# cosdata/cosdata

Measured on AMD Instinct MI355X. Metric: QPS at recall@10≥0.95, 1024-dim dense cosine, 1/2/4/8 MI355X, higher is better.
Workload: dtype u8

## Files before the change

cosdata_amd/_lib.py:

```python
from __future__ import annotations

import ctypes as C
import os
import subprocess

_PKG = os.path.dirname(os.path.abspath(__file__))
SO_PATH = os.path.join(_PKG, "libcosdata_hip.so")
CSRC = os.path.join(_PKG, "csrc")

OK, ERR_STORAGE_MISMATCH, ERR_CALCULATION, ERR_INVALID, ERR_UNIMPLEMENTED, ERR_HIP, ERR_NOT_READY, ERR_NO_DEVICE = range(8)
STATUS_NAMES = {
    0: "OK", 1: "StorageMismatch", 2: "CalculationError", 3: "Invalid", 4: "Unimplemented", 5: "HipError",
    6: "NotReady", 7: "NoDevice",
}
ABI_VERSION = 1


class CosdataError(RuntimeError):

    def __init__(self, status: int, message: str):
        super().__init__(f"[{STATUS_NAMES.get(status, status)}] {message}")
        self.status = status


class CosParams(C.Structure):
    _fields_ = [
        ("struct_size", C.c_uint32), ("abi_version", C.c_uint32), ("dim", C.c_uint32), ("metric", C.c_uint32),
        ("storage", C.c_uint32), ("resolution", C.c_uint32), ("range_lo", C.c_float), ("range_hi", C.c_float),
        ("num_layers", C.c_uint32), ("neighbors_count", C.c_uint32), ("level0_neighbors_count", C.c_uint32),
        ("ef_construction", C.c_uint32), ("ef_search", C.c_uint32), ("shortlist_size", C.c_uint32),
        ("visited_mode", C.c_uint32), ("device", C.c_int32), ("id_base", C.c_uint32), ("reserved", C.c_uint32),
        ("seed", C.c_uint64),
    ]


class CosSearchStats(C.Structure):
    _fields_ = [
        ("evals", C.c_uint64), ("expansions", C.c_uint64), ("adj_bytes", C.c_uint64), ("rerank_rows", C.c_uint64),
        ("walk_ms", C.c_float), ("finalize_ms", C.c_float), ("prep_ms", C.c_float), ("reserved", C.c_uint32),
    ]


class CosWalkSplit(C.Structure):
    _fields_ = [
        ("struct_size", C.c_uint32), ("queries", C.c_uint32), ("table_level_min", C.c_uint32), ("table_cols", C.c_uint32),
        ("cut_after_level", C.c_uint32), ("reserved", C.c_uint32),
        ("table_ms", C.c_float), ("upper_ms", C.c_float), ("sort_ms", C.c_float), ("lower_ms", C.c_float),
        ("table_int8_ops", C.c_double), ("table_evals", C.c_uint64),
        ("upper_evals", C.c_uint64), ("upper_expansions", C.c_uint64), ("upper_adj_bytes", C.c_uint64),
        ("lower_evals", C.c_uint64), ("lower_expansions", C.c_uint64), ("lower_adj_bytes", C.c_uint64),
    ]


class CosTimingSummary(C.Structure):
    _fields_ = [("launches", C.c_uint32), ("prep_ms_sum", C.c_float), ("walk_ms_sum", C.c_float), ("finalize_ms_sum", C.c_float),
                ("walk_ms_min", C.c_float), ("walk_ms_max", C.c_float)]


class CosCoalescingStats(C.Structure):
    _fields_ = [("launches", C.c_uint64), ("queries", C.c_uint64), ("requests", C.c_uint64), ("closed_full", C.c_uint64),
                ("closed_quiet", C.c_uint64), ("closed_deadline", C.c_uint64), ("solo_calls", C.c_uint64)]


class CosSparseStats(C.Structure):
    _fields_ = [("kernel_ms", C.c_float), ("blocks", C.c_uint32), ("postings_visited", C.c_uint64), ("posting_bytes", C.c_uint64)]


class CosFlatStats(C.Structure):
    _fields_ = [("gemm_ms", C.c_float), ("gemm_launches", C.c_uint32), ("int8_ops", C.c_double), ("code_bytes", C.c_double)]


class CosBM25Stats(C.Structure):
    _fields_ = [("struct_size", C.c_uint32), ("documents_count", C.c_uint32), ("n_terms", C.c_uint32), ("largest_doc_id", C.c_uint32),
                ("dir_rows", C.c_uint32), ("dir_tiles", C.c_uint32), ("reserved", C.c_uint32),
                ("postings", C.c_uint64), ("tombstones", C.c_uint64), ("device_bytes", C.c_uint64)]


class CosSparseIndexStats(C.Structure):
    _fields_ = [("struct_size", C.c_uint32), ("n_vectors", C.c_uint32), ("n_dims", C.c_uint32), ("dir_rows", C.c_uint32),
                ("dir_tiles", C.c_uint32), ("packed", C.c_uint32), ("have_raw", C.c_uint32), ("reserved", C.c_uint32),
                ("postings", C.c_uint64), ("removed", C.c_uint64), ("raw_pairs", C.c_uint64), ("device_bytes", C.c_uint64)]


def build(force: bool = False, verbose: bool = False) -> str:
    srcs = [os.path.join(CSRC, f) for f in os.listdir(CSRC) if f.endswith((".hip", ".h"))]
    srcs.append(os.path.join(_PKG, "..", "include", "cosdata_hip.h"))
    stale = force or not os.path.exists(SO_PATH) or any(os.path.getmtime(s) > os.path.getmtime(SO_PATH) for s in srcs)
    if force:
        subprocess.check_call(["make", "-C", CSRC, "-s", "clean"])
    if stale:
        cmd = ["make", "-C", CSRC, "-j", str(max(2, min(16, 2 * (os.cpu_count() or 1))))]
        if not verbose:
            cmd.append("-s")
        subprocess.check_call(cmd)
    return SO_PATH


_lib = None

ABI_SYMBOLS = [
    "cos_index_create", "cos_index_destroy", "cos_last_error_string", "cos_device_count",
    "cos_index_upload_vectors", "cos_index_set_root", "cos_index_upload_graph_level", "cos_index_level_count",
    "cos_index_download_graph_level", "cos_index_download_codes", "cos_index_download_root", "cos_index_build", "cos_index_append", "cos_index_delete", "cos_index_restore_link_state", "cos_index_release_link_state", "cos_index_enable_metadata", "cos_index_upload_meta_nodes", "cos_index_upload_meta_graph_level", "cos_index_build_meta", "cos_index_meta_level_count", "cos_index_download_meta_graph_level", "cos_search_filtered_batch",
    "cos_ann_search_filtered_batch", "cos_index_load_reference_dir", "cos_reference_dir_level_counts", "cos_reference_dir_read_level",
    "cos_search_batch", "cos_search_batch_device", "cos_ann_search_batch", "cos_index_set_coalescing", "cos_index_coalescing_stats", "cos_index_set_ef_search",
    "cos_index_set_visited_mode", "cos_index_set_latency_mode", "cos_index_set_latency_waves", "cos_index_set_walk_order", "cos_index_walk_order_cuts", "cos_index_set_walk_table", "cos_index_walk_table_info", "cos_index_last_walk_split", "cos_index_enable_timing", "cos_index_last_stats", "cos_index_timing_summary", "cos_quantize_batch",
    "cos_code_bytes", "cos_sample_values_range", "cos_distance_batch", "cos_bruteforce_topk", "cos_flat_search_batch", "cos_bm25_create", "cos_bm25_destroy",
    "cos_bm25_insert", "cos_bm25_delete", "cos_bm25_stats", "cos_bm25_download",
    "cos_bm25_search_batch", "cos_bm25_search_batch_device", "cos_rrf_fuse_batch", "cos_hybrid_search_batch", "cos_text_process", "cos_text_count_tokens", "cos_bm25_term_frequency", "cos_xxhash32", "cos_stem_english", "cos_sparse_create", "cos_sparse_build_csr", "cos_sparse_create_from_vectors", "cos_sparse_destroy", "cos_sparse_search_batch", "cos_sparse_last_stats", "cos_sparse_layout",
    "cos_sparse_set_max_candidates", "cos_sparse_max_candidates",
    "cos_sparse_insert", "cos_sparse_delete", "cos_sparse_stats", "cos_sparse_download", "cos_merge_topk_device", "cos_merge_topk_packed_device", "cos_hbm_probe",
    "cos_shardset_unique_id", "cos_shardset_create", "cos_shardset_destroy", "cos_shardset_search_batch", "cos_shardset_exchange_device",
    "cos_tuning_set", "cos_tuning_clear", "cos_tuning_get",
]


def lib():
    global _lib
    if _lib is not None:
        return _lib
    if not os.path.exists(SO_PATH):
        raise CosdataError(ERR_NO_DEVICE, f"{SO_PATH} is missing: build it with `python -c 'import __graft_entry__ as g; g.build()'` "
                                          "(the HIP extension is mandatory; there is no CPU path)")
    try:
        import torch
    except ImportError:
        pass
    L = C.CDLL(SO_PATH)
    vp, i32, u32, f32 = C.c_void_p, C.c_int32, C.c_uint32, C.c_float
# ... 150 lines not shown
```

cosdata_amd/csrc/engine.hip:

```cpp
#include <hip/hip_runtime.h>

#include <algorithm>
#include <cstdarg>
#include <cstdio>
#include <cstdlib>
#include <chrono>
#include <cmath>
#include <condition_variable>
#include <cstring>
#include <map>
#include <mutex>
#include <string>
#include <thread>
#include <vector>

#include "engine_internal.h"

using namespace cosdev;

static thread_local std::string g_err;
int32_t cos_fail(int32_t code, const char *fmt, ...) {
    char buf[512];
    va_list ap;
    va_start(ap, fmt);
// ... 572 lines not shown
    if (!vt.zeroed) {
        HIP_TRY(hipMemsetAsync(vt.bits, 0, vt.bits.cap * 4, st));
        vt.zeroed = true;
    }
    wa.vis_bits = vt.bits;
    wa.vis_log = vt.log;
    wa.vis_words_per_query = words;
    wa.vis_log_cap = (u32)log_cap;
    return COS_OK;
}

static int32_t ensure_order_rank(cos_index *ix) {
    if (ix->order_rank_valid) return COS_OK;
    for (u32 l = 0; l < cosdev::MAX_LEVELS; l++) {
        ix->d_order_rank[l].reset();
        ix->order_rank_n[l] = 0;
    }
    ix->order_levels.clear();
    const u32 Ltop = ix->p.num_layers;
    auto usable = [&](u32 l) { return l >= 1 && l <= Ltop && ix->lv[l].n > 1 && ix->lv[l].n <= (1u << 20) && ix->lv[l].d_adj_node; };
    std::vector<u32> want;
    if (const long long mask = cosdev::tune(cosdev::TUNE_WALK_SPLIT_LEVELS); mask != cosdev::TUNE_UNSET) {
        for (u32 l = Ltop; l >= 1; l--)
            if ((mask >> l) & 1) want.push_back(l);
    } else {
        for (u32 l = 1; l <= Ltop; l++)
            if (usable(l) && (size_t)ix->lv[l].n * ix->row_stride <= ((size_t)64 << 20)) { want.push_back(l); break; }
    }
    u32 prev = Ltop + 1;
    for (u32 l : want) {
        if (!usable(l) || l >= prev) continue;
        ix->order_levels.push_back(l);
        prev = l;
    }
    if (!ix->order_levels.empty()) HIP_TRY(hipDeviceSynchronize());
    for (u32 kl : ix->order_levels) {
        const LevelHost &H = ix->lv[kl];
        const u32 n = H.n, M = H.M;
        std::vector<u32> adj((size_t)n * M), rank(n, 0u), stack;
        HIP_TRY(hipMemcpy(adj.data(), H.d_adj_node, adj.size() * 4, hipMemcpyDeviceToHost));
        std::vector<uint8_t> seen(n, 0);
        u32 next = 0;
        auto dfs_from = [&](u32 start) {
            stack.push_back(start);
            while (!stack.empty()) {
                const u32 v = stack.back();
                stack.pop_back();
                if (seen[v]) continue;
                seen[v] = 1;
                rank[v] = next++;
                const u32 *row = &adj[(size_t)v * M];
                for (u32 j = M; j-- > 0;) {
                    const u32 u = row[j];
                    if (u != cosdev::ROW_EMPTY && u < n && !seen[u]) stack.push_back(u);
                }
            }
        };
        dfs_from(n - 1);
        for (u32 v = 0; v < n; v++) if (!seen[v]) dfs_from(v);
        HIP_TRY(ix->d_order_rank[kl].alloc(n));
        HIP_TRY(hipMemcpy(ix->d_order_rank[kl], rank.data(), (size_t)n * 4, hipMemcpyHostToDevice));
        ix->order_rank_n[kl] = n;
    }
    ix->order_rank_valid = true;
    return COS_OK;
}

static void clear_current_table(cos_index *ix) {
    ix->d_tcodes = nullptr;
    ix->d_tmags = nullptr;
    ix->d_tcsums = nullptr;
    ix->table_cols = 0;
    ix->table_level_min = 0;
    ix->table_stride = 0;
}
static u32 walk_table_max_cols(const cos_index *ix) {
    const long long env = cosdev::tune_or(cosdev::TUNE_WALK_TABLE_COLS, -1);
    return env >= 0 ? (u32)std::min<long long>(env, 1ll << 20) : ix->walk_table_max_cols;
}
static u32 walk_table_min_B(const cos_index *ix) {
    const long long env = cosdev::tune_or(cosdev::TUNE_WALK_TABLE_MIN_B, -1);
    return env >= 0 ? (u32)std::min<long long>(env, 0xFFFFFFFFll) : ix->walk_table_min_B;
}
cosdev::WalkPlanIn cos_walk_plan_in(const cos_index *ix, u32 B, u32 ef) {
    cosdev::WalkPlanIn in{};
    in.eng = ix->eng;
    in.storage = ix->p.storage;
    in.nchunks = ix->nchunks;
    in.G = ix->G;
    in.num_layers = ix->p.num_layers;
    for (u32 l = 0; l <= ix->p.num_layers; l++) in.M[l] = ix->lv[l].M;
    in.shortlist = ix->p.shortlist_size;
    in.visited_mode = ix->p.visited_mode;
    in.mdim = ix->meta.mdim;
    in.B = B;
    in.ef = ef;
    in.chain = true;
    const long long lat = cosdev::tune_or(cosdev::TUNE_WALK_LAT, -1), lat4 = cosdev::tune_or(cosdev::TUNE_WALK_LAT4, -1);
    in.lat_max_B = lat >= 0 ? (u32)std::min(lat, 0xFFFFFFFFll) : ix->lat_max_B;
    in.lat4_max_B = lat4 >= 0 ? (u32)std::min(lat4, 0xFFFFFFFFll) : ix->lat4_max_B;
    in.small_table_tk = cosdev::tune_or(cosdev::TUNE_WALK_SMALL_TABLE_TK, 1) != 0;
    in.adj_mag_mode = (u32)cosdev::tune_or(cosdev::TUNE_WALK_ADJ_MAG, 1);
    in.table_min_B = walk_table_min_B(ix);
    in.order_min_B = ix->walk_order_min_B;
    in.chain_min_B = ix->chain_min_B;
    in.side_min_B = ix->walk_side_min_B;
    in.table_after_sort = cosdev::tune_or(cosdev::TUNE_WALK_TABLE_AFTER_SORT, 1);
    in.table_supported = cosdev::level_table_eng_supported(ix->eng, ix->row_stride);
    in.adj_mag_valid = ix->adj_mag_valid;
    return in;
}
static int32_t ensure_level_table(cos_index *ix) {
    const u32 max_cols = walk_table_max_cols(ix);
    const bool automatic = max_cols == COS_WALK_TABLE_AUTO;
    const u32 efs = ix->p.ef_search, Mup = ix->p.neighbors_count;
    const u64 c_rule = (u64)cosdev::tune_or(cosdev::TUNE_WALK_TABLE_RULE_C, 2u * efs <= 3u * Mup ? 10 : (efs <= 2u * Mup ? 8 : 6));
    const u64 per_level = automatic ? std::min<u64>(c_rule * ix->p.ef_search * ix->p.neighbors_count, 1u << 20) : (u64)(1u << 20);
    const u64 total_cap = automatic ? (u64)(1u << 20) : (u64)max_cols;
    const u64 key = automatic ? (0x8000000000000000ull | per_level) : (u64)max_cols;
    if (ix->level_table_valid && ix->table_built_for_key == key) return COS_OK;
    if (!ix->level_table_valid) {
        HIP_TRY(hipDeviceSynchronize());
        ix->table_sets.clear();
    }
    ix->level_table_valid = true;
    ix->table_built_for_key = key;
    clear_current_table(ix);
    for (const auto &t : ix->table_sets)
        if (t.key == key) {
            ix->table_level_min = t.level_min;
            ix->table_cols = t.cols;
            ix->table_stride = t.stride;
            memcpy(ix->table_col0, t.col0, sizeof(t.col0));
            ix->d_tcodes = t.tcodes;
            ix->d_tmags = t.tmags;
            ix->d_tcsums = t.tcsums;
            return COS_OK;
        }
    if (!cosdev::level_table_eng_supported(ix->eng, ix->row_stride) || max_cols == 0) return COS_OK;
    const u32 Ltop = ix->p.num_layers;
    u32 cols = 0, lmin = 0;
    for (u32 l = Ltop; l >= 1; l--) {
        if (!ix->lv[l].d_node_vec || ix->lv[l].n == 0 || ix->lv[l].n > per_level || (u64)cols + ix->lv[l].n > total_cap) break;
        cols += ix->lv[l].n;
        lmin = l;
    }
    if (lmin == 0) return COS_OK;
    HIP_TRY(hipDeviceSynchronize());
    cos_index::TableSet t;
    auto build = [&]() -> hipError_t {
        hipError_t e = t.tcodes.alloc((size_t)cols * ix->row_stride);
        if (e == hipSuccess) e = t.tmags.alloc(cols);
        if (e == hipSuccess) e = t.tcsums.alloc(cols);
        u32 c0 = 0;
        for (u32 l = Ltop; l >= lmin && e == hipSuccess; l--) {
            ix->table_col0[l] = c0;
            e = cosdev::launch_level_table_gather(ix->d_codes, ix->d_mags, ix->row_stride, ix->lv[l].d_node_vec, ix->lv[l].n, c0, t.tcodes, t.tmags, nullptr);
            c0 += ix->lv[l].n;
        }
        if (e == hipSuccess) e = cosdev::launch_code_sums(t.tcodes, ix->row_stride, cols, t.tcsums, nullptr);
        if (e == hipSuccess) e = hipDeviceSynchronize();
        return e;
    };
    if (const hipError_t e = build(); e != hipSuccess) {
        (void)hipDeviceSynchronize();
        if (e == hipErrorOutOfMemory) {
            (void)hipGetLastError();
            return COS_OK;
        }
        ix->level_table_valid = false;
        HIP_TRY(e);
    }
    ix->d_tcodes = t.tcodes;
    ix->d_tmags = t.tmags;
    ix->d_tcsums = t.tcsums;
    ix->table_cols = cols;
    ix->table_level_min = lmin;
    ix->table_stride = ((u64)cols + 31) / 32 * 32;
    t.key = key;
    t.level_min = lmin;
    t.cols = cols;
    t.stride = ix->table_stride;
    memcpy(t.col0, ix->table_col0, sizeof(t.col0));
    ix->table_sets.push_back(std::move(t));
    return COS_OK;
}

extern "C" int32_t cos_index_set_walk_table(cos_index *ix, uint32_t max_cols, uint32_t min_queries) {
    if (!ix) return cos_fail(COS_ERR_INVALID, "null argument");
    if (max_cols > (1u << 20) && max_cols != COS_WALK_TABLE_AUTO) return cos_fail(COS_ERR_INVALID, "max_cols must be <= 2^20 (or COS_WALK_TABLE_AUTO)");
    std::lock_guard<std::mutex> g(ix->mu);
    ix->walk_table_max_cols = max_cols;
// ... 20 lines not shown
    if (!graph_ready(ix) || ix->meta.mdim != 0u) return COS_OK;
    if (cosdev::walk_rows_over_64_slots(cos_walk_plan_in(ix, 0, 0))) return COS_OK;
    HIP_TRY(hipDeviceSynchronize());
    for (u32 l = 0; l <= ix->p.num_layers; l++) {
        ix->lv[l].d_adj_mag.reset();
    }
    for (u32 l = 0; l <= ix->p.num_layers; l++) {
        LevelHost &H = ix->lv[l];
        const u32 slots = std::min(H.M, ix->p.shortlist_size);
        const hipError_t e = H.d_adj_mag.alloc((size_t)H.n * slots);
        if (e == hipErrorOutOfMemory) {
            (void)hipGetLastError();
            for (u32 k = 0; k < l; k++) ix->lv[k].d_adj_mag.reset();
            return COS_OK;
        }
        HIP_TRY(e);
        HIP_TRY(cosdev::launch_fill_adj_mag(H.d_adj_vec, ix->d_mags, H.d_adj_mag, H.n, H.M, slots, ix->own_stream));
    }
    HIP_TRY(hipStreamSynchronize(ix->own_stream));
    ix->adj_mag_valid = true;
    return COS_OK;
}

int32_t cos_prepare_walk_plans(cos_index *ix) {
    std::lock_guard<std::mutex> g(ix->mu);
    if (int32_t rc = ensure_adj_mags(ix)) return rc;
    if (ix->walk_order_min_B)
        if (int32_t rc = ensure_order_rank(ix)) return rc;
    if (walk_table_min_B(ix))
        if (int32_t rc = ensure_level_table(ix)) return rc;
    return COS_OK;
}

extern "C" int32_t cos_index_walk_order_cuts(cos_index *ix, uint32_t *out_levels, uint32_t cap, uint32_t *out_n) {
    if (!ix || !out_n || (cap && !out_levels)) return cos_fail(COS_ERR_INVALID, "null argument");
    *out_n = 0;
    if (!graph_ready(ix)) return cos_fail(COS_ERR_NOT_READY, "index needs vectors, root and every graph level");
    int32_t rc = cos_set_device(ix);
    if (rc) return rc;
    std::lock_guard<std::mutex> g(ix->mu);
    if ((rc = ensure_order_rank(ix))) return rc;
    for (u32 l : ix->order_levels) {
        if (*out_n < cap) out_levels[*out_n] = l;
        (*out_n)++;
    }
    return COS_OK;
}

struct SearchLaunch {
    cosdev::WalkPlan plan;
    u32 ef = 0, visited_mode = 0;
    bool timed = false;
    u64 tab_stride = 0;
    u32 tab_col0[cosdev::MAX_LEVELS] = {};
    const uint8_t *tcodes = nullptr;
    const float *tmags = nullptr;
    const u32 *tcsums = nullptr;
    u32 n_keys = 0, key_level[cosdev::MAX_LEVELS], key_n[cosdev::MAX_LEVELS];
    const u32 *order_rank[cosdev::MAX_LEVELS];
};

static int32_t get_workspace(cos_index *ix, void *key, hipStream_t st, u32 B, u32 top_k, bool host_api, Workspace **out, SearchLaunch *L,
                             bool chain = true) {
    std::lock_guard<std::mutex> g(ix->mu);
    std::unique_ptr<Workspace> &slot = ix->ws[key];
    if (!slot) slot.reset(new Workspace());
    Workspace *w = slot.get();
    const u32 L1 = ix->p.num_layers + 1;
    if (B > w->capB) {
        u32 cap = std::max(B, 64u);
        HIP_TRY(hipStreamSynchronize(st));
        w->capB = 0;
        w->cap_topk = 0;
        HIP_TRY(w->q_codes.alloc((size_t)cap * ix->row_stride));
        HIP_TRY(w->q_mags.alloc(cap));
        HIP_TRY(w->q_raw_mags.alloc(cap));
        HIP_TRY(w->walk_ids.alloc((size_t)cap * L1 * KEEP_SEARCH));
        HIP_TRY(w->walk_sims.alloc((size_t)cap * L1 * KEEP_SEARCH));
        HIP_TRY(w->walk_counts.alloc((size_t)cap * L1));
        HIP_TRY(w->walk_status.alloc(cap));
        HIP_TRY(w->stats.alloc((size_t)cap * 4));
        HIP_TRY(w->stats2.alloc((size_t)cap * 4));
        HIP_TRY(w->qsums.alloc(cap));
        if (ix->eng == ENG_Q2) HIP_TRY(w->qdig.alloc((size_t)cap * (ix->row_stride / 16) * 64));
        HIP_TRY(w->fin_flags.alloc((size_t)cap + 1));
        HIP_TRY(w->rerank_rows.alloc(cap));
        HIP_TRY(w->d_queries.alloc((size_t)cap * ix->p.dim));
        HIP_TRY(w->d_out_counts.alloc(cap));
        HIP_TRY(w->d_out_status.alloc(cap));
        w->capB = cap;
    }
    L->ef = ix->p.ef_search;
    L->visited_mode = ix->p.visited_mode;
    L->timed = ix->timing;
    cosdev::WalkPlanIn in = cos_walk_plan_in(ix, B, L->ef);
    in.chain = chain;
    const cosdev::WalkPlan want = cosdev::walk_plan(in);
    cosdev::WalkHave have{};
    if (want.refill_adj_mag) {
        if (int32_t rc = ensure_adj_mags(ix)) return rc;
        in.adj_mag_valid = ix->adj_mag_valid;
    }
    if (want.prepare_order) {
        if (w->order.cap < w->capB) {
            HIP_TRY(hipStreamSynchronize(st));
            HIP_TRY(cosdev::walk_order_reserve(w->order, w->capB));
        }
        if (int32_t rc = ensure_order_rank(ix)) return rc;
        have.order_buffers = w->order.cap >= B;
        have.n_order_keys = (u32)ix->order_levels.size();
        have.order_level0 = have.n_order_keys ? ix->order_levels[0] : 0u;
    }
    if (want.prepare_table) {
        if (int32_t rc = ensure_level_table(ix)) return rc;
        const size_t need = (size_t)w->capB * ix->table_stride;
        if (need > w->tab.cap) {
            const size_t budget = (size_t)cosdev::tune_or(cosdev::TUNE_WALK_TABLE_MAX_BYTES, (long long)48 << 30);
            HIP_TRY(hipStreamSynchronize(st));
            ix->table_bytes_total -= w->tab.cap * 4;
            w->tab.reset();
            if (ix->table_bytes_total + need * 4 <= budget) {
                if (const hipError_t e = w->tab.alloc(need); e == hipSuccess)
                    ix->table_bytes_total += need * 4;
                else if (e == hipErrorOutOfMemory)
                    (void)hipGetLastError();
                else
                    HIP_TRY(e);
            }
        }
        have.table_level_min = ix->level_table_valid ? ix->table_level_min : 0u;
        have.table_cols = ix->table_cols;
        have.table_buffer = w->tab && (size_t)B * ix->table_stride <= w->tab.cap;
    }
    L->plan = cosdev::walk_plan(in, &have);
    if (L->plan.use_table) {
        L->tab_stride = ix->table_stride;
        memcpy(L->tab_col0, ix->table_col0, sizeof(L->tab_col0));
        L->tcodes = ix->d_tcodes;
        L->tmags = ix->d_tmags;
        L->tcsums = ix->d_tcsums;
    }
    if (L->plan.ordered)
        for (u32 l : ix->order_levels) {
            L->key_level[L->n_keys] = l;
            L->key_n[L->n_keys] = ix->order_rank_n[l];
            L->order_rank[L->n_keys++] = ix->d_order_rank[l];
        }
    if (host_api && (size_t)top_k * w->capB > (size_t)w->cap_topk * w->capB) {
        w->cap_topk = 0;
        HIP_TRY(w->d_out_ids.alloc((size_t)w->capB * top_k));
        HIP_TRY(w->d_out_scores.alloc((size_t)w->capB * top_k));
        w->cap_topk = top_k;
    }
    if (w->ev.empty()) {
        w->ev.assign((size_t)Workspace::EV_RING * Workspace::EV_PER, nullptr);
        for (auto &e : w->ev) HIP_TRY(hipEventCreate(&e));
    }
    if (!w->walk_done) HIP_TRY(hipEventCreateWithFlags(&w->walk_done, hipEventDisableTiming));
    if (!w->walk_fin) HIP_TRY(hipEventCreateWithFlags(&w->walk_fin, hipEventDisableTiming));
    if (!w->last_range) HIP_TRY(hipEventCreateWithFlags(&w->last_range, hipEventDisableTiming));
    *out = w;
    return COS_OK;
}

static int32_t run_search(cos_index *ix, Workspace *w, const SearchLaunch &L, const float *d_queries, u32 B, u32 top_k, u32 *d_out_ids,
                          float *d_out_scores, u32 *d_out_counts, int32_t *d_out_status, bool do_finalize, hipStream_t st,
                          hipStream_t st_fin = nullptr, hipEvent_t walk_ev = nullptr) {
    const cosdev::WalkPlan &plan = L.plan;
    const bool timed = L.timed, ordered = plan.ordered, chained = plan.chained;
    const u32 ef = L.ef, n_keys = L.n_keys;
    IndexDev dev = cos_make_index_dev(ix);
    dev.visited_mode = L.visited_mode;
    for (u32 l = 0; l <= dev.num_layers; l++)
        if (!((plan.use_adj_mag >> l) & 1u)) dev.lv[l].adj_mag = nullptr;
    WalkArgs wa;
    memset(&wa, 0, sizeof(wa));
    if (dev.visited_mode == COS_VISITED_EXACT) {
        int32_t rc = vis_tab_prepare(w->vis, ix, B, ef, st, wa);
        if (rc) return rc;
    }
    hipEvent_t *ev = &w->ev[(size_t)(w->ev_count % Workspace::EV_RING) * Workspace::EV_PER];
    if (timed) HIP_TRY(hipEventRecord(ev[0], st));
    HIP_TRY(launch_quantize_rows(ix->eng, d_queries, ix->p.dim, B, ix->p.dim, ix->p.range_lo, ix->p.range_hi, w->q_codes, ix->row_stride,
                                 w->q_mags, w->q_raw_mags, st));
    if (plan.use_table) {
        if (plan.table_waits_for_sort) {
            std::lock_guard<std::mutex> g(ix->chain_mu);
            if (ix->chain_last_range_ev && ix->chain_last_range_ev != w->last_range) HIP_TRY(hipStreamWaitEvent(st, ix->chain_last_range_ev, 0));
        }
        if (timed) HIP_TRY(hipEventRecord(ev[4], st));
        HIP_TRY(cosdev::launch_level_table(ix->eng, w->q_codes, w->q_mags, w->qsums, w->qdig, B, L.tcodes, L.tmags, L.tcsums, ix->row_stride, plan.table_cols,
                                           w->tab, L.tab_stride, ix->n_cus, st));
        if (timed) HIP_TRY(hipEventRecord(ev[5], st));
    }
    if (timed) HIP_TRY(hipEventRecord(ev[1], st));
    wa.qcodes = w->q_codes;
    wa.qmags = w->q_mags;
    wa.B = B;
    wa.ef = ef;
    wa.keep = KEEP_SEARCH;
    wa.out_ids = w->walk_ids;
    wa.out_sims = w->walk_sims;
    wa.out_counts = w->walk_counts;
    wa.out_status = w->walk_status;
    wa.out_stats = w->stats;
    wa.out_stats2 = w->stats2;
    HIP_TRY(hipMemsetAsync(w->stats2, 0, (size_t)B * 32, st));
    if (plan.use_table) {
        wa.tab = w->tab;
        wa.tab_mags = L.tmags;
        wa.tab_stride = L.tab_stride;
        wa.tab_level_min = plan.table_level_min;
        memcpy(wa.tab_col0, L.tab_col0, sizeof(L.tab_col0));
    }
    hipStream_t sw = st;
    if (plan.side_stream) {
        if (!w->walk_stream) {
            int lo = 0, hi = 0;
            HIP_TRY(hipDeviceGetStreamPriorityRange(&lo, &hi));
            HIP_TRY(hipStreamCreateWithPriority(&w->walk_stream, hipStreamNonBlocking, lo));
            HIP_TRY(hipEventCreateWithFlags(&w->prep_done, hipEventDisableTiming));
        }
        sw = w->walk_stream;
        HIP_TRY(hipEventRecord(w->prep_done, st));
        HIP_TRY(hipStreamWaitEvent(sw, w->prep_done, 0));
    }
    auto walk = [&](hipStream_t s) -> int32_t {
        if (!ordered) {
            if (chained) HIP_TRY(hipEventRecord(w->last_range, s));
            HIP_TRY(launch_walk(ix->eng, dev, wa, plan.kernel, s));
            return COS_OK;
        }
        wa.phase = 1;
        wa.entry0 = w->order.entry0;
        wa.order_key = w->order.order_key;
        wa.order_iota = w->order.iota;
        u32 first = dev.num_layers;
        for (u32 i = 0; i <= n_keys; i++) {
            const bool last = i == n_keys;
            wa.level_first = first;
            wa.level_last = last ? 0u : L.key_level[i];
            wa.key_n = last ? 0u : L.key_n[i];
            wa.order_rank = last ? nullptr : L.order_rank[i];
            if (last && chained) HIP_TRY(hipEventRecord(w->last_range, s));
            HIP_TRY(launch_walk(ix->eng, dev, wa, plan.kernel, s));
            if (last) break;
            if (timed && i == 0) HIP_TRY(hipEventRecord(ev[6], s));
            HIP_TRY(cosdev::launch_walk_order(w->order, B, L.key_n[i], ix->num_xcd, s));
            if (timed && i == 0) HIP_TRY(hipEventRecord(ev[7], s));
            wa.q_order = w->order.q_order;
            first = L.key_level[i] - 1;
        }
        return COS_OK;
    };
    if (chained) {
        std::lock_guard<std::mutex> g(ix->chain_mu);
        if (ix->chain_ev && ix->chain_ev != w->walk_done) HIP_TRY(hipStreamWaitEvent(sw, ix->chain_ev, 0));
        if (timed) HIP_TRY(hipEventRecord(ev[1], sw));
        if (int32_t rc = walk(sw)) return rc;
        HIP_TRY(hipEventRecord(w->walk_done, sw));
        ix->chain_ev = w->walk_done;
        ix->chain_last_range_ev = w->last_range;
    } else {
        if (timed && sw != st) HIP_TRY(hipEventRecord(ev[1], sw));
        if (int32_t rc = walk(sw)) return rc;
    }
    if (timed) HIP_TRY(hipEventRecord(ev[2], sw));
    hipStream_t sf = st_fin ? st_fin : st;
    if (sf != sw) {
        hipEvent_t we = walk_ev ? walk_ev : w->walk_fin;
        HIP_TRY(hipEventRecord(we, sw));
        HIP_TRY(hipStreamWaitEvent(sf, we, 0));
    }
    if (do_finalize) {
        HIP_TRY(launch_finalize(dev, d_queries, ix->p.dim, w->q_raw_mags, w->walk_ids, w->walk_sims, w->walk_counts, w->walk_status, B, top_k,
                                d_out_ids, d_out_scores, d_out_counts, d_out_status, w->rerank_rows, sf, ordered ? w->order.q_order : nullptr, w->fin_flags));
    }
    if (timed) { HIP_TRY(hipEventRecord(ev[3], sf)); w->ev_count++; }
    w->lastB = B;
    w->timed = timed;
    w->last_plan = plan;
    { std::lock_guard<std::mutex> g(ix->mu); ix->last_ws = w; }
    return COS_OK;
}

static int32_t check_search_args(cos_index *ix, const void *q, u32 B, u32 top_k) {
    if (!ix || !q) return cos_fail(COS_ERR_INVALID, "null argument");
    if (!graph_ready(ix)) return cos_fail(COS_ERR_NOT_READY, "index needs vectors, root and every graph level before search");
    if (top_k == 0 || top_k > 1024) return cos_fail(COS_ERR_INVALID, "top_k must be in [1, 1024]");
    if (B == 0) return cos_fail(COS_ERR_INVALID, "empty batch");
    return cos_set_device(ix);
}

extern "C" int32_t cos_search_batch_device(cos_index *ix, const float *d_queries, uint32_t B, uint32_t top_k, uint32_t *d_out_ids,
                                           float *d_out_scores, uint32_t *d_out_counts, int32_t *d_out_status, void *stream) {
    int32_t rc = check_search_args(ix, d_queries, B, top_k);
    if (rc) return rc;
    if (!d_out_ids || !d_out_scores || !d_out_counts || !d_out_status) return cos_fail(COS_ERR_INVALID, "null output");
    Workspace *w;
    SearchLaunch L;
    rc = get_workspace(ix, stream, (hipStream_t)stream, B, top_k, false, &w, &L);
    if (rc) return rc;
    return run_search(ix, w, L, d_queries, B, top_k, d_out_ids, d_out_scores, d_out_counts, d_out_status, true, (hipStream_t)stream);
}

struct PipeLease {
    cos_index *ix;
    HostPipe *hp = nullptr;
    explicit PipeLease(cos_index *ix_) : ix(ix_) {}
    PipeLease(const PipeLease &) = delete;
    PipeLease &operator=(const PipeLease &) = delete;
    int32_t acquire() {
        std::unique_lock<std::mutex> lk(ix->pipe_mu);
        for (;;) {
            if (!ix->pipes_free.empty()) { hp = ix->pipes_free.back(); ix->pipes_free.pop_back(); break; }
            if (ix->pipes_all.size() < COS_MAX_HOST_PIPES) {
                std::unique_ptr<HostPipe> n(new HostPipe());
                hipError_t e = hipStreamCreateWithFlags(&n->s[0], hipStreamNonBlocking);
                if (e != hipSuccess) return cos_fail(COS_ERR_HIP, "hipStreamCreateWithFlags: %s", hipGetErrorString(e));
                hp = n.get();
                ix->pipes_all.push_back(std::move(n));
                break;
            }
            ix->pipe_cv.wait(lk);
        }
        ix->host_calls_active.fetch_add(1);
        return COS_OK;
    }
    ~PipeLease() {
        if (!hp) return;
        ix->host_calls_active.fetch_sub(1);
        { std::lock_guard<std::mutex> g(ix->pipe_mu); ix->pipes_free.push_back(hp); }
        ix->pipe_cv.notify_one();
    }
};

static int32_t report_status(const int32_t *status, u32 B) {
    for (u32 b = 0; b < B; b++)
        if (status[b] != COS_OK) return cos_fail(status[b], "query %u failed with status %d (zero-norm vector -> DistanceError::CalculationError)", b, status[b]);
    return COS_OK;
}

static int32_t search_host_simple(cos_index *ix, HostPipe *hp, const float *queries, uint32_t B, uint32_t top_k, uint32_t *out_ids, float *out_scores,
                                  uint32_t *out_counts, int32_t *out_status) {
    hipStream_t st = hp->s[0];
// ... 302 lines not shown
    if (rc) return rc;
    if (!out_ids || !out_sims || !out_counts) return cos_fail(COS_ERR_INVALID, "null output");
    PipeLease lease(ix);
    rc = lease.acquire();
    if (rc) return rc;
    hipStream_t st = lease.hp->s[0];
    Workspace *w;
    SearchLaunch L;
    rc = get_workspace(ix, (void *)st, st, B, 1, true, &w, &L);
    if (rc) return rc;
    const u32 L1 = ix->p.num_layers + 1;
    HIP_TRY(hipMemcpyAsync(w->d_queries, queries, (size_t)B * ix->p.dim * 4, hipMemcpyHostToDevice, st));
    rc = run_search(ix, w, L, w->d_queries, B, 1, nullptr, nullptr, nullptr, nullptr, false, st);
    if (rc) return rc;
    std::vector<int32_t> status(B);
    HIP_TRY(hipMemcpyAsync(out_ids, w->walk_ids, (size_t)B * L1 * KEEP_SEARCH * 4, hipMemcpyDeviceToHost, st));
    HIP_TRY(hipMemcpyAsync(out_sims, w->walk_sims, (size_t)B * L1 * KEEP_SEARCH * 4, hipMemcpyDeviceToHost, st));
    HIP_TRY(hipMemcpyAsync(out_counts, w->walk_counts, (size_t)B * L1 * 4, hipMemcpyDeviceToHost, st));
    HIP_TRY(hipMemcpyAsync(status.data(), w->walk_status, (size_t)B * 4, hipMemcpyDeviceToHost, st));
    HIP_TRY(hipStreamSynchronize(st));
    if (out_status) memcpy(out_status, status.data(), (size_t)B * 4);
    for (u32 b = 0; b < B; b++)
        if (status[b] != COS_OK) return cos_fail(status[b], "query %u failed with status %d", b, status[b]);
    return COS_OK;
}

static Workspace *find_workspace(cos_index *ix, void *stream, bool null_is_last) {
    std::lock_guard<std::mutex> g(ix->mu);
    if (!stream && null_is_last) return ix->last_ws;
    auto it = ix->ws.find(stream);
    return it != ix->ws.end() ? it->second.get() : nullptr;
}
static int32_t sum_launch_stats(const u64 *d_stats, u32 B, u64 sum[4]) {
    std::vector<u64> st((size_t)B * 4);
    HIP_TRY(hipMemcpy(st.data(), d_stats, st.size() * 8, hipMemcpyDeviceToHost));
    sum[0] = sum[1] = sum[2] = sum[3] = 0;
    for (u32 b = 0; b < B; b++)
        for (int k = 0; k < 4; k++) sum[k] += st[(size_t)b * 4 + k];
    return COS_OK;
}

extern "C" int32_t cos_index_last_stats(cos_index *ix, void *stream, cos_search_stats *out) {
    if (!ix || !out) return cos_fail(COS_ERR_INVALID, "null argument");
    memset(out, 0, sizeof(*out));
    int32_t rc = cos_set_device(ix);
    if (rc) return rc;
    Workspace *w = find_workspace(ix, stream, true);
    if (!w || w->lastB == 0) return cos_fail(COS_ERR_NOT_READY, "no batch has run on this stream");
    if (w->timed && w->ev_count) {
        hipEvent_t *ev = &w->ev[(size_t)((w->ev_count - 1) % Workspace::EV_RING) * Workspace::EV_PER];
        HIP_TRY(hipEventSynchronize(ev[3]));
        HIP_TRY(hipEventElapsedTime(&out->prep_ms, ev[0], ev[1]));
        HIP_TRY(hipEventElapsedTime(&out->walk_ms, ev[1], ev[2]));
        HIP_TRY(hipEventElapsedTime(&out->finalize_ms, ev[2], ev[3]));
    } else {
        HIP_TRY(hipDeviceSynchronize());
    }
    u64 st[4];
    if ((rc = sum_launch_stats(w->stats, w->lastB, st))) return rc;
    out->evals = st[0];
    out->expansions = st[1];
    out->adj_bytes = st[2];
    out->reserved = (uint32_t)st[3];
    std::vector<u64> rr(w->lastB);
    HIP_TRY(hipMemcpy(rr.data(), w->rerank_rows, rr.size() * 8, hipMemcpyDeviceToHost));
    for (u32 b = 0; b < w->lastB; b++) out->rerank_rows += rr[b];
    return COS_OK;
}

extern "C" int32_t cos_index_last_walk_split(cos_index *ix, void *stream, cos_walk_split *out) {
    if (!ix || !out) return cos_fail(COS_ERR_INVALID, "null argument");
    if (out->struct_size != sizeof(cos_walk_split)) return cos_fail(COS_ERR_INVALID, "cos_walk_split.struct_size mismatch");
    memset(out, 0, sizeof(*out));
    out->struct_size = sizeof(cos_walk_split);
    int32_t rc = cos_set_device(ix);
    if (rc) return rc;
    Workspace *w = find_workspace(ix, stream, true);
    if (!w || w->lastB == 0) return cos_fail(COS_ERR_NOT_READY, "no batch has run on this stream");
    const cosdev::WalkPlan &plan = w->last_plan;
    out->queries = w->lastB;
    out->table_level_min = plan.table_level_min;
    out->table_cols = plan.table_cols;
    out->cut_after_level = plan.cut_after_level;
    if (w->timed && w->ev_count) {
        hipEvent_t *ev = &w->ev[(size_t)((w->ev_count - 1) % Workspace::EV_RING) * Workspace::EV_PER];
        HIP_TRY(hipEventSynchronize(ev[3]));
        if (plan.use_table) HIP_TRY(hipEventElapsedTime(&out->table_ms, ev[4], ev[5]));
        if (plan.ordered) {
            HIP_TRY(hipEventElapsedTime(&out->upper_ms, ev[1], ev[6]));
            HIP_TRY(hipEventElapsedTime(&out->sort_ms, ev[6], ev[7]));
            HIP_TRY(hipEventElapsedTime(&out->lower_ms, ev[7], ev[2]));
        } else
            HIP_TRY(hipEventElapsedTime(&out->lower_ms, ev[1], ev[2]));
    } else {
        HIP_TRY(hipDeviceSynchronize());
    }
    const u32 kdims = (u32)((ix->row_stride + 63) / 64 * 64);
    out->table_int8_ops = 2.0 * (double)w->lastB * (double)out->table_cols * (double)kdims;
    u64 st[4], s2[4];
    if ((rc = sum_launch_stats(w->stats, w->lastB, st)) || (rc = sum_launch_stats(w->stats2, w->lastB, s2))) return rc;
    out->lower_evals = s2[0];
    out->lower_expansions = s2[1];
    out->lower_adj_bytes = s2[2];
    out->table_evals = s2[3];
    out->upper_evals = st[0] - s2[0];
    out->upper_expansions = st[1] - s2[1];
    out->upper_adj_bytes = st[2] - s2[2];
    return COS_OK;
}

extern "C" int32_t cos_index_timing_summary(cos_index *ix, void *stream, cos_timing_summary *out) {
    if (!ix || !out) return cos_fail(COS_ERR_INVALID, "null argument");
    memset(out, 0, sizeof(*out));
    int32_t rc = cos_set_device(ix);
    if (rc) return rc;
    Workspace *w = find_workspace(ix, stream, false);
    if (!w || w->ev_count == 0) return cos_fail(COS_ERR_NOT_READY, "no timed batch has run on this stream");
    const u32 n = std::min(w->ev_count, Workspace::EV_RING);
    out->launches = n;
    out->walk_ms_min = 1e30f;
    for (u32 i = 0; i < n; i++) {
        hipEvent_t *ev = &w->ev[(size_t)((w->ev_count - 1 - i) % Workspace::EV_RING) * Workspace::EV_PER];
        float a = 0, b = 0, c = 0;
        HIP_TRY(hipEventSynchronize(ev[3]));
        HIP_TRY(hipEventElapsedTime(&a, ev[0], ev[1]));
        HIP_TRY(hipEventElapsedTime(&b, ev[1], ev[2]));
        HIP_TRY(hipEventElapsedTime(&c, ev[2], ev[3]));
        out->prep_ms_sum += a;
        out->walk_ms_sum += b;
        out->finalize_ms_sum += c;
        out->walk_ms_min = std::min(out->walk_ms_min, b);
        out->walk_ms_max = std::max(out->walk_ms_max, b);
    }
    return COS_OK;
}

static constexpr u32 PSEUDO_LO = 0xFFFFFEFEu, PSEUDO_HI = 0xFFFFFFFDu;

extern "C" int32_t cos_index_enable_metadata(cos_index *ix, uint32_t mdim, uint32_t max_replicas_per_node) {
    if (!ix || mdim == 0 || mdim > 64 || max_replicas_per_node == 0) return cos_fail(COS_ERR_INVALID, "metadata dimensions must be in [1, 64] and max_replicas_per_node >= 1");
    if (!ix->have_vectors) return cos_fail(COS_ERR_NOT_READY, "upload vectors before enabling the metadata component");
    if (ix->p.ef_construction > cosdev::WALK_FAST_MAX_EF || std::min(ix->p.neighbors_count, ix->p.shortlist_size) > 64u ||
        std::min(ix->p.level0_neighbors_count, ix->p.shortlist_size) > 64u ||
        (ix->nchunks != 0u && (ix->nchunks + ix->G - 1u) / ix->G > (ix->eng == ENG_U8 ? 2u : 1u)))
        return cos_fail(COS_ERR_UNIMPLEMENTED, "metadata collections: ef_construction <= %u, at most 64 scanned neighbour slots per node, u8 rows of at most 2048 / SubByte rows of at most 64 x 16 bytes", cosdev::WALK_FAST_MAX_EF);
    if ((u64)ix->n * max_replicas_per_node >= PSEUDO_LO) return cos_fail(COS_ERR_INVALID, "replica ids would run into the reserved id range");
    if (ix->p.id_base % max_replicas_per_node != 0)
        return cos_fail(COS_ERR_INVALID, "id_base %u of a metadata collection's shard must be a multiple of max_replicas_per_node %u (first embedding x replicas)", ix->p.id_base, max_replicas_per_node);
    if ((u64)ix->p.id_base + (u64)ix->n * max_replicas_per_node >= PSEUDO_LO) return cos_fail(COS_ERR_INVALID, "replica ids would run into the reserved id range");
    for (auto &l : ix->lv)
        if (l.n) return cos_fail(COS_ERR_INVALID, "enable the metadata component before uploading / building the base graph: it changes the id of every vector (row x max_replicas)");
    int32_t rc = cos_set_device(ix);
    if (rc) return rc;
    ix->id_stride = max_replicas_per_node;
    ix->meta.mdim = mdim;
    ix->meta.lv.resize(ix->p.num_layers + 1);
    for (u32 l = 0; l <= ix->p.num_layers; l++) ix->meta.lv[l].M = l == 0 ? ix->p.level0_neighbors_count : ix->p.neighbors_count;
    DevBuf z;
    HIP_TRY(z.alloc(((size_t)ix->p.dim + 1) * 4));
    HIP_TRY(hipMemsetAsync(z.p, 0, ((size_t)ix->p.dim + 1) * 4, ix->own_stream));
    HIP_TRY(launch_quantize_rows(ix->eng, z.as<float>(), ix->p.dim, 1, ix->p.dim, ix->p.range_lo, ix->p.range_hi,
                                 ix->d_codes + ((size_t)ix->n + 1) * ix->row_stride, ix->row_stride, ix->d_mags + ix->n + 1, z.as<float>() + ix->p.dim, ix->own_stream));
    HIP_TRY(hipStreamSynchronize(ix->own_stream));
    return COS_OK;
}

extern "C" int32_t cos_index_upload_meta_nodes(cos_index *ix, uint32_t n_nodes, const uint32_t *node_ids, const int32_t *mbits) {
    if (!ix || !node_ids || !mbits || n_nodes == 0) return cos_fail(COS_ERR_INVALID, "null/empty node table");
    if (!ix->meta.mdim || !ix->have_vectors) return cos_fail(COS_ERR_NOT_READY, "cos_index_enable_metadata first");
    int32_t rc = cos_set_device(ix);
// ... 239 lines not shown
```

cosdata_amd/csrc/engine_internal.h:

```cpp
#pragma once
#include <hip/hip_runtime.h>

#include <atomic>
#include <condition_variable>
#include <map>
#include <memory>
#include <mutex>
#include <string>
#include <thread>
#include <vector>

#include "../../include/cosdata_hip.h"
#include "engine_types.h"
#include "tuning.h"
#include "link_types.h"
#include "dev_mem.h"
#include "walk_plan.h"

namespace cosdev {
hipError_t launch_fill_i32(int32_t *p, u64 n, int32_t v, hipStream_t st);
hipError_t launch_edge_pairs(const u32 *adj_vec, const u32 *node_vec, u32 node0, u32 cn, u32 M, u32 *px, u32 *py, hipStream_t st);
hipError_t launch_edge_keys(const u32 *adj_vec, const float *sims, const int32_t *st_in, u32 node0, u32 cn, u32 M, u32 metric, int32_t *key, int32_t *fail, hipStream_t st);
hipError_t launch_low_cache(const u32 *adj_vec, const int32_t *key, u32 n, u32 M, int32_t kmin, int32_t kmax, uint8_t *low_idx, int32_t *low_key, hipStream_t st);
hipError_t launch_unlink(const LinkArgs &a, const u32 *dn, u32 *status, hipStream_t st);
hipError_t launch_index_pair_distances(int eng, const uint8_t *codes, const float *mags, u64 row_stride, u32 nchunks, u32 dim, u32 metric, const u32 *d_pair_x,
                                       const u32 *d_pair_y, u32 n_pairs, float *d_out, int32_t *d_status, hipStream_t st);
hipError_t launch_grow_rows(const u32 *src, u32 *dst, u32 old_n, u32 new_n, u32 M, u32 remap_from, u32 remap_to, u32 fill, hipStream_t st);
hipError_t launch_grow_bytes(const uint8_t *src, uint8_t *dst, u32 old_n, u32 new_n, hipStream_t st);
hipError_t launch_fill_adj_mag(const u32 *adj_vec, const float *mags, float *adj_mag, u32 n, u32 M, u32 slots, hipStream_t st);
hipError_t launch_link_round(const LinkArgs &a, u32 maxM, const u32 *pend, const u32 *pcount, u32 *next, u32 *next_count, u32 *evq, u32 *evq_count,
                             u32 count_ub, u32 round, hipStream_t st);
hipError_t launch_quantize_rows(int eng, const float *x, u64 x_stride, u32 n, u32 dim, float lo, float hi, uint8_t *codes,
                                u64 row_stride, float *mags, float *raw_mags, hipStream_t st);
hipError_t launch_walk(int eng, const IndexDev &ix, const WalkArgs &wa, WalkKernel kernel, hipStream_t st);
static_assert(WALK_PLAN_MAX_LEVELS == MAX_LEVELS && WALK_PLAN_ENG_U8 == ENG_U8 && WALK_PLAN_ENG_Q2 == ENG_Q2 && WALK_PLAN_FAST_MAX_EF == WALK_FAST_MAX_EF &&
              COS_STORAGE_U8 == 0u && COS_VISITED_REF == 0u, "walk_plan.h restates these");
hipError_t launch_walk_meta(int eng, const IndexDev &ix, const WalkArgs &wa, hipStream_t st);
hipError_t launch_walk_meta_index(int eng, const IndexDev &ix, const WalkArgs &wa, hipStream_t st);
hipError_t launch_finalize(const IndexDev &ix, const float *queries, u64 q_stride, const float *q_raw_mags, const u32 *walk_ids,
                           const float *walk_sims, const u32 *walk_counts, const int32_t *walk_status, u32 B, u32 top_k,
                           u32 *out_ids, float *out_scores, u32 *out_counts, int32_t *out_status, u64 *out_rerank_rows,
                           hipStream_t st, const u32 *q_order = nullptr, u32 *slow_list = nullptr);
struct WalkOrder {
    u32 cap = 0;
    DevArr<u32> entry0;
    DevArr<u32> order_key;
    DevArr<u32> keys_sorted;
    DevArr<u32> iota, vals_sorted, q_order;
    DevBuf tmp;
};
hipError_t walk_order_reserve(WalkOrder &o, u32 B);
hipError_t launch_walk_order(WalkOrder &o, u32 B, u32 key_max, u32 num_xcd, hipStream_t st);
hipError_t launch_level_table_gather(const uint8_t *codes, const float *mags, u64 row_stride, const u32 *node_vec, u32 n, u32 col0,
                                     uint8_t *tcodes, float *tmags, hipStream_t st);
hipError_t launch_code_sums(const uint8_t *codes, u64 row_stride, u32 n, u32 *sums, hipStream_t st);
hipError_t launch_level_table(int eng, const uint8_t *qcodes, const float *qmags, u32 *qsums, uint8_t *qdig, u32 B, const uint8_t *tcodes, const float *tmags,
                              const u32 *tcsums, u64 row_stride, u32 ncols, float *tab, u64 tab_stride, u32 n_cus, hipStream_t st);
bool level_table_eng_supported(int eng, u64 row_stride);
int32_t quantize_ref_layout(uint32_t storage, uint32_t res, uint32_t dim, const float *x, uint32_t n, void *codes, float *mags);
int32_t distance_ref_layout(uint32_t metric, uint32_t storage, uint32_t res, uint32_t dim, const void *x_codes, const float *x_mags, uint32_t nx,
                            const void *y_codes, const float *y_mags, uint32_t ny, const uint32_t *pair_x, const uint32_t *pair_y, uint32_t n_pairs,
                            float *out, int32_t *status);
}

using cosdev::u32;
using cosdev::u64;

int32_t cos_fail(int32_t code, const char *fmt, ...);
#define HIP_TRY(expr)                                                                                  \
    do {                                                                                               \
        hipError_t _e = (expr);                                                                        \
        if (_e != hipSuccess) return cos_fail(COS_ERR_HIP, "%s: %s (%s:%d)", #expr, hipGetErrorString(_e), __FILE__, __LINE__); \
    } while (0)

struct LevelHost {
    std::vector<u32> node_ids;
    std::vector<u32> nbr_ids;
    DevArr<u32> d_adj_vec, d_adj_node, d_node_vec, d_child;
    DevArr<u32> d_node_id, d_node_meta;
    DevArr<float> d_adj_mag;
    u32 n = 0, M = 0;
    u32 root_idx = 0;
    bool host_valid = false;
    void release() {
        d_adj_vec.reset(); d_adj_node.reset(); d_node_vec.reset(); d_child.reset();
        d_node_id.reset(); d_node_meta.reset(); d_adj_mag.reset();
        n = 0;
        node_ids.clear();
        nbr_ids.clear();
        host_valid = false;
    }
};

struct LinkState {
    DevBuf key[cosdev::MAX_LEVELS], low_idx[cosdev::MAX_LEVELS], low_key[cosdev::MAX_LEVELS], owner[cosdev::MAX_LEVELS];
    uint64_t rng = 0;
    u32 n_built = 0;
    bool valid = false;
    void release() {
        for (int l = 0; l < cosdev::MAX_LEVELS; l++) { key[l].reset(); low_idx[l].reset(); low_key[l].reset(); owner[l].reset(); }
        valid = false;
    }
};

struct VisTab {
    DevArr<u32> bits, log;
    bool zeroed = false;
};
int32_t vis_tab_prepare(VisTab &vt, const cos_index *ix, u32 B, u32 ef, hipStream_t st, cosdev::WalkArgs &wa);

struct Workspace {
    u32 capB = 0, cap_topk = 0;
    DevArr<uint8_t> q_codes;
    DevArr<float> q_mags, q_raw_mags;
    DevArr<u32> walk_ids, walk_counts;
    DevArr<float> walk_sims;
    DevArr<int32_t> walk_status;
    DevArr<u64> stats;
    DevArr<u64> stats2;
    DevArr<float> tab;
    DevArr<u32> qsums;
    DevArr<uint8_t> qdig;
    DevArr<u32> fin_flags;
    DevArr<u64> rerank_rows;
    VisTab vis;
    cosdev::WalkOrder order;
    DevArr<float> d_queries;
    DevArr<u32> d_out_ids, d_out_counts;
    DevArr<float> d_out_scores;
    DevArr<int32_t> d_out_status;
    DevArr<u32> f_buf;
    static constexpr u32 EV_RING = 128;
    static constexpr u32 EV_PER = 8;
    std::vector<hipEvent_t> ev;
    u32 ev_count = 0;
    hipEvent_t walk_done = nullptr;
    hipEvent_t last_range = nullptr;
    hipStream_t walk_stream = nullptr;
    hipEvent_t prep_done = nullptr, walk_fin = nullptr;
    u32 lastB = 0;
    bool timed = false;
    cosdev::WalkPlan last_plan{};
    Workspace() = default;
    Workspace(const Workspace &) = delete;
    ~Workspace() {
        for (hipEvent_t e : {walk_done, walk_fin, last_range, prep_done}) if (e) (void)hipEventDestroy(e);
        for (hipEvent_t e : ev) if (e) (void)hipEventDestroy(e);
        if (walk_stream) (void)hipStreamDestroy(walk_stream);
    }
};

struct MetaGraph {
    u32 mdim = 0;
    std::vector<u32> node_ids;
    DevArr<int32_t> d_mbits;
    DevArr<float> d_mmags;
    std::vector<LevelHost> lv;
};

struct HostPipe {
    static constexpr u32 MAX_CHUNKS = 4;
    hipStream_t s[2] = {nullptr, nullptr}, sc = nullptr, sf = nullptr;
    hipEvent_t ev_in[MAX_CHUNKS] = {}, ev_walk[MAX_CHUNKS] = {};
    char wkey[MAX_CHUNKS] = {};
    DevArr<float> d_q;
    DevArr<u32> d_ids, d_counts;
    DevArr<float> d_scores;
    DevArr<int32_t> d_status;
    HostPipe() = default;
    HostPipe(const HostPipe &) = delete;
    ~HostPipe() {
        for (hipEvent_t e : ev_in) if (e) (void)hipEventDestroy(e);
        for (hipEvent_t e : ev_walk) if (e) (void)hipEventDestroy(e);
        for (hipStream_t st : {s[0], s[1], sc, sf}) if (st) (void)hipStreamDestroy(st);
    }
};
static constexpr u32 COS_MAX_HOST_PIPES = 32;

struct cos_index {
    cos_params p;
    int eng = -1;
    u32 n = 0;
    bool have_vectors = false, have_root = false;
    const float *d_raw = nullptr;
    DevArr<float> raw_own;
    DevArr<float> d_raw_mags;
    DevArr<uint8_t> d_codes;
    DevArr<float> d_mags;
    u64 row_stride = 0;
    u32 nchunks = 0, G = 1;
    std::vector<float> root_raw;
    std::vector<LevelHost> lv;
    u32 id_stride = 1;
    MetaGraph meta;
    hipStream_t own_stream = nullptr;
    std::mutex mu;
    std::map<void *, std::unique_ptr<Workspace>> ws;
    std::mutex pipe_mu;
    std::condition_variable pipe_cv;
    std::vector<std::unique_ptr<HostPipe>> pipes_all;
    std::vector<HostPipe *> pipes_free;
    std::atomic<int> host_calls_active{0};
    Workspace *last_ws = nullptr;
    std::mutex co_mu;
    std::condition_variable co_cv;
    std::vector<struct CoSlot *> co_slots;
    struct CoSlot *co_open = nullptr;
    u32 co_max_queries = 0, co_window_us = 0;
    u32 co_inflight = 0;
    cos_coalescing_stats co_stats{};
    bool timing = false;
    std::mutex chain_mu;
    hipEvent_t chain_ev = nullptr;
    hipEvent_t chain_last_range_ev = nullptr;
    u32 chain_min_B = 16384;
    u32 walk_order_min_B = COS_WALK_ORDER_DEFAULT_MIN_B;
    u32 n_cus = 256;
    u32 num_xcd = 8;
    DevArr<u32> d_order_rank[cosdev::MAX_LEVELS];
    u32 order_rank_n[cosdev::MAX_LEVELS] = {};
    std::vector<u32> order_levels;
    bool order_rank_valid = false;
    u32 walk_table_max_cols = COS_WALK_TABLE_AUTO, walk_table_min_B = COS_WALK_TABLE_DEFAULT_MIN_B;
    size_t table_bytes_total = 0;
    bool adj_mag_valid = false;
    LinkState link;
    bool level_table_valid = false;
    u32 table_level_min = 0, table_cols = 0;
    u64 table_built_for_key = 0;
    u64 table_stride = 0;
    u32 table_col0[cosdev::MAX_LEVELS] = {};
    const uint8_t *d_tcodes = nullptr;
    const float *d_tmags = nullptr;
    const u32 *d_tcsums = nullptr;
    struct TableSet { u64 key; u32 level_min, cols; u64 stride; u32 col0[cosdev::MAX_LEVELS]; DevArr<uint8_t> tcodes; DevArr<float> tmags; DevArr<u32> tcsums; };
    std::vector<TableSet> table_sets;
    u32 walk_side_min_B = 4096;
    u32 lat_max_B = COS_LATENCY_MODE_DEFAULT_MAX_B;
    u32 lat4_max_B = COS_LATENCY_WAVES_DEFAULT_MAX_B;
    struct FlatWs *flat_ws = nullptr;
};


struct FlatWs;
void cos_flat_ws_release(cos_index *ix);
void cos_coalesce_release(cos_index *ix);
cosdev::IndexDev cos_make_index_dev(const cos_index *ix);
cosdev::IndexDev cos_make_meta_dev(const cos_index *ix);
int32_t cos_set_device(const cos_index *ix);
cosdev::WalkPlanIn cos_walk_plan_in(const cos_index *ix, u32 B, u32 ef);
int32_t cos_prepare_walk_plans(cos_index *ix);
void cos_meta_free_levels(cos_index *ix);
```

cosdata_amd/csrc/flat_scan.h:

```cpp
#pragma once
#include <hip/hip_runtime.h>

#include "engine_types.h"

namespace cosdev {

struct FusedOut {
    const u64 *thr;
    u64 *app;
    u32 *app_cnt;
    u32 cap;
    const uint8_t *qdigits;
};


bool flat_scan_supported(u32 kdims);
hipError_t launch_flat_scan_expand_queries(const uint8_t *qcodes, u64 row_stride, u32 B, u32 kdims, uint8_t *digits, hipStream_t st, bool fp4);
hipError_t launch_flat_scan(u32 kdims, u32 n_cus, hipStream_t st, const uint8_t *qdig, const float *qmags, u32 B, const uint8_t *codes,
                            const float *mags, u64 row_stride, u32 n0, u32 nc, u32 metric, const FusedOut &fo, bool fp4);

hipError_t launch_flat_scan_u8(u32 kdims, u32 n_cus, hipStream_t st, const uint8_t *qcodes, const u32 *qsums, const float *qmags, u32 B, const uint8_t *codes,
                               const u32 *csums, const float *mags, u64 row_stride, u32 n0, u32 nc, u32 metric, const FusedOut &fo);

constexpr u32 FLAT_SEED = 16384;
__host__ __device__ constexpr u32 flat_growth(u32 P) { return P == 64 ? 8u : 4u; }
__host__ __device__ constexpr u32 flat_app_cap(u32 P) { return P == 64 ? 4096u : 32u * P; }
inline u32 flat_pool_width(u32 need) {
    for (u32 P = 64; P <= 1024; P *= 2)
        if (need <= P) return P;
    return 0;
}
hipError_t launch_flat_select_wide(u32 R, const float *d_scores, u64 s_stride, u32 B, u32 n0, u32 nc, u64 *d_part, u32 S, u64 *d_pool, u64 *d_thr,
                                   hipStream_t st);
hipError_t launch_flat_append_wide(u32 R, const u64 *d_app, u32 *d_appcnt, u32 cap, u32 B, u64 *d_pool, u64 *d_thr, u32 *d_overflow, hipStream_t st);
hipError_t launch_flat_rerank_wide(u32 R, bool brute, const float *Q, u64 q_stride, const float *qmags, u32 B, const float *X, u64 x_stride,
                                   const float *xmags, u32 dim, const u64 *d_pool, u32 ncand_max, u32 k, u32 id_base, u32 *out_ids, float *out_scores,
                                   u32 *out_counts, hipStream_t st);

bool level_table_areg_supported(int eng, u64 row_stride);
hipError_t launch_level_table_areg(int eng, u32 n_cus, hipStream_t st, const uint8_t *qcodes, const u32 *qsums, u32 B, const uint8_t *tcodes,
                                   const u32 *tcsums, u64 row_stride, u32 ncols, float *tab, u64 tab_stride);

}
```

cosdata_amd/csrc/kernels_flat.hip:

```cpp
#include <hip/hip_runtime.h>

#include <algorithm>
#include <cstdlib>
#include <cstring>
#include <type_traits>
#include <vector>

#include "dot_engines.h"
#include "engine_internal.h"
#include "flat_scan.h"
#include "topk_select.h"

using namespace cosdev;

namespace {

typedef float f32x16 __attribute__((ext_vector_type(16)));

constexpr int BM = 128, BN = 128, BK = 32, LDT = BK + 4;
constexpr int SEL = 64;
constexpr size_t GEMM_SMEM = 2ull * (BM + BN) * LDT * sizeof(float);

template <bool VEC, bool FUSED>
__global__ __launch_bounds__(256) void flat_gemm_f32(const float *__restrict__ Q, u64 q_stride, const float *__restrict__ qmags, u32 B,
// ... 772 lines not shown
            streamed += (double)nc * (double)ix->row_stride * (double)((B + CM - 1) / CM);
            n0 += nc;
            seen += nc;
        }
        const size_t nk = (size_t)B * top_k, out_words = 2 * nk + B + 2;
        if (e == hipSuccess) e = W->out.grow(out_words);
        if (e == hipSuccess) e = W->h_out.grow(out_words);
        if (e != hipSuccess) break;
        if (R == 1) {
            hipLaunchKernelGGL(flat_rerank_top5k, dim3(B), dim3(64), (((size_t)dim * 4 + 15) & ~(size_t)15), st, d_q, (u64)dim, d_qrm, B, ix->d_raw, (u64)dim,
                               ix->d_raw_mags, dim, d_pool, 5 * top_k, top_k, ix->p.id_base, d_oi, d_os, d_oc);
        } else {
            e = launch_flat_rerank_wide(R, false, d_q, (u64)dim, d_qrm, B, ix->d_raw, (u64)dim, ix->d_raw_mags, dim, d_pool, 5 * top_k, top_k, ix->p.id_base,
                                        d_oi, d_os, d_oc, st);
            if (e != hipSuccess) break;
        }
        hipLaunchKernelGGL(flat_pack_out_kernel, dim3((u32)((std::max<size_t>(nk, B) + 255) / 256)), dim3(256), 0, st, d_oi, d_os, d_oc, d_zero, B, top_k, W->out.p);
        e = hipGetLastError();
        if (e == hipSuccess) e = hipMemcpyAsync(W->h_out, W->out.p, out_words * 4, hipMemcpyDeviceToHost, st);
        if (e == hipSuccess) e = hipStreamSynchronize(st);
        if (e != hipSuccess) break;
        const u32 *ho = W->h_out;
        zero = ho[2 * nk + B] != 0;
        const u32 hover = ho[2 * nk + B + 1];
        if (zero) break;
        if (fused && hover != 0) continue;
        memcpy(out_ids, ho, nk * 4);
        memcpy(out_scores, ho + nk, nk * 4);
        memcpy(out_counts, ho + 2 * nk, (size_t)B * 4);
        break;
    }
    if (e == hipSuccess && !zero) {
        for (size_t i = 0; i + 1 < n_ev && e == hipSuccess; i += 2) {
            float ms = 0.f;
            e = hipEventElapsedTime(&ms, W->evs[i], W->evs[i + 1]);
            gemm_ms += ms;
        }
    }
    if (stats) {
        stats->gemm_ms = gemm_ms;
        stats->gemm_launches = launches;
        stats->int8_ops = 2.0 * (double)B * (double)n * (double)kdims;
        stats->code_bytes = streamed;
    }
    HIP_TRY(e);
    if (zero) return cos_fail(COS_ERR_CALCULATION, "zero-norm query or stored vector: DistanceError::CalculationError (cosine.rs:228-232)");
    return COS_OK;
}

namespace {
__global__ __launch_bounds__(256) void level_table_gather_kernel(const uint8_t *__restrict__ codes, const float *__restrict__ mags, u64 row_stride,
                                                                 const u32 *__restrict__ node_vec, u32 n, u32 col0, uint8_t *__restrict__ tcodes,
                                                                 float *__restrict__ tmags) {
    const int lane = threadIdx.x & 63;
    const u32 node = blockIdx.x * 4 + (threadIdx.x >> 6);
    if (node >= n) return;
    const u32 row = node_vec[node];
    const uint4 *src = (const uint4 *)(codes + (u64)row * row_stride);
    uint4 *dst = (uint4 *)(tcodes + (u64)(col0 + node) * row_stride);
    for (u32 c = lane; c < (u32)(row_stride / 16); c += 64) dst[c] = src[c];
    if (lane == 0) tmags[col0 + node] = mags[row];
}
}

namespace cosdev {

hipError_t launch_level_table_gather(const uint8_t *codes, const float *mags, u64 row_stride, const u32 *node_vec, u32 n, u32 col0,
                                     uint8_t *tcodes, float *tmags, hipStream_t st) {
    if (n == 0) return hipSuccess;
    hipLaunchKernelGGL(level_table_gather_kernel, dim3((n + 3) / 4), dim3(256), 0, st, codes, mags, row_stride, node_vec, n, col0, tcodes, tmags);
    return hipGetLastError();
}

hipError_t launch_code_sums(const uint8_t *codes, u64 row_stride, u32 n, u32 *sums, hipStream_t st) {
    if (n == 0) return hipSuccess;
    hipLaunchKernelGGL(code_sums_kernel, dim3((n + 3) / 4), dim3(256), 0, st, codes, row_stride, n, sums);
    return hipGetLastError();
}

bool level_table_eng_supported(int eng, u64 row_stride) {
    return eng == ENG_U8 || (eng == ENG_Q2 && level_table_areg_supported(ENG_Q2, row_stride));
}

hipError_t launch_level_table(int eng, const uint8_t *qcodes, const float *qmags, u32 *qsums , uint8_t *qdig ,
                              u32 B, const uint8_t *tcodes, const float *tmags, const u32 *tcsums, u64 row_stride, u32 ncols, float *tab, u64 tab_stride,
                              u32 n_cus, hipStream_t st) {
    if (B == 0 || ncols == 0) return hipSuccess;
    const bool q2 = eng == ENG_Q2;
    const u32 kdims = q2 ? (u32)(row_stride / 16) * 64 : (u32)((row_stride + 63) / 64 * 64);
    hipError_t e = hipSuccess;
    if (!q2) e = launch_code_sums(qcodes, row_stride, B, qsums, st);
    if (e != hipSuccess) return e;
    if (level_table_areg_supported(eng, row_stride) && tune_or(TUNE_WALK_TABLE_GEMM, 1) != 0) {
        if (q2) {
            e = launch_flat_scan_expand_queries(qcodes, row_stride, B, kdims, qdig, st, false);
            if (e != hipSuccess) return e;
        }
        return launch_level_table_areg(eng, n_cus ? n_cus : 256u, st, q2 ? qdig : qcodes, (const u32 *)qsums, B, tcodes, tcsums, row_stride, ncols, tab, tab_stride);
    }
    const u32 metric = 1u;
    dim3 grid((ncols + CN - 1) / CN, (B + CM - 1) / CM);
    FusedOut fo{nullptr, nullptr, nullptr, 0u, nullptr};
    if (q2)
        hipLaunchKernelGGL((flat_codes_gemm_i8<ENG_Q2, false, 2>), grid, dim3(512), 0, st, qcodes, qmags, (const u32 *)qsums, B, tcodes, tmags, tcsums, row_stride, 0u,
                           ncols, kdims, metric, tab, tab_stride, fo);
    else
        hipLaunchKernelGGL((flat_codes_gemm_i8<ENG_U8, false, 2>), grid, dim3(512), 0, st, qcodes, qmags, (const u32 *)qsums, B, tcodes, tmags, tcsums, row_stride, 0u,
                           ncols, kdims, metric, tab, tab_stride, fo);
    return hipGetLastError();
}

}
```

cosdata_amd/csrc/kernels_scan.hip:

```cpp
#include <hip/hip_runtime.h>

#include <algorithm>
#include <cstdlib>
#include <type_traits>

#include "device_common.h"
#include "flat_scan.h"
#include "tuning.h"

using namespace cosdev;

namespace {

typedef int i32x4 __attribute__((ext_vector_type(4)));
typedef int i32x16 __attribute__((ext_vector_type(16)));

__device__ __forceinline__ u32 q2_dword_perm(uint4 raw , int pp, int jj) {
    const u32 w0 = pp < 2 ? raw.x : raw.y, w1 = pp < 2 ? raw.z : raw.w;
    const int sh = 4 * (pp & 1) + jj;
    const u32 x0 = w0 >> sh, x1 = sh ? (w1 >> (sh - 1)) : (w1 << 1);
    return (x0 & 0x01010101u) | (x1 & 0x02020202u);
}
__device__ __forceinline__ uint4 q2_piece_perm(uint4 raw, int pp) {
    return make_uint4(q2_dword_perm(raw, pp, 0), q2_dword_perm(raw, pp, 1), q2_dword_perm(raw, pp, 2), q2_dword_perm(raw, pp, 3));
}

__global__ void expand_q2_digits_perm_kernel(const uint8_t *__restrict__ qcodes, u64 row_stride, u32 B, u32 kdims, uint8_t *__restrict__ digits) {
    const u64 t = (u64)blockIdx.x * blockDim.x + threadIdx.x;
    const u32 chunks = kdims / 64;
    if (t >= (u64)B * chunks) return;
    const u32 q = (u32)(t / chunks), j = (u32)(t % chunks);
    const uint4 raw = (u64)j * 16 < row_stride ? *(const uint4 *)(qcodes + (u64)q * row_stride + (u64)j * 16) : make_uint4(0, 0, 0, 0);
#pragma unroll
    for (int pp = 0; pp < 4; pp++) *(uint4 *)(digits + (u64)q * kdims + (u64)j * 64 + pp * 16) = q2_piece_perm(raw, pp);
}

template <bool FIRST>
__device__ __forceinline__ void areg_mfma(i32x16 &acc, const i32x4 &afrag, const i32x4 &bfrag) {
    const i32x16 z = {0, 0, 0, 0, 0, 0, 0, 0, 0, 0, 0, 0, 0, 0, 0, 0};
    acc = __builtin_amdgcn_mfma_i32_32x32x32_i8(afrag, bfrag, FIRST ? z : acc, 0, 0, 0);
}

constexpr int AREG_STAGE = 2048;

__device__ __forceinline__ void areg_append(const FusedOut &fo, const float *__restrict__ qmags, const float *__restrict__ mags, u32 metric, u32 n0,
                                            u32 col, u32 row, u32 dot) {
    const float dotf = (float)dot;
    const float sc = metric == 0u ? __fdiv_rn(dotf, __fmul_rn(qmags[row], mags[n0 + col])) : dotf;
    const u64 key = pack_key(simkey(sc), n0 + col);
    if (key > fo.thr[row]) {
        const u32 pos = atomicAdd(&fo.app_cnt[row], 1u);
        if (pos < fo.cap) fo.app[(u64)row * fo.cap + pos] = key;
    }
}

template <int I, int N, class F>
__device__ __forceinline__ void static_for(F &&f) {
    if constexpr (I < N) {
        f(std::integral_constant<int, I>{});
        static_for<I + 1, N>(f);
    }
}

template <int KC>
__global__ __launch_bounds__(256) void flat_scan_q2_areg(const uint8_t *__restrict__ qdig ,
                                                         const float *__restrict__ qmags, u32 B, const uint8_t *__restrict__ codes,
                                                         const float *__restrict__ mags, u64 row_stride, u32 n0, u32 n_chunk, u32 metric,
                                                         const FusedOut fo) {
    constexpr int K = KC * 64, KS = KC * 2, LDB = K + 16, ITS = (KC + 3) / 4, PIECES = ITS * 4;
    extern __shared__ __attribute__((aligned(16))) unsigned char areg_lds[];
    u32 *stage = (u32 *)(areg_lds + (size_t)2 * 64 * LDB), *stage_cnt = stage + 3 * AREG_STAGE;
    const int tid = threadIdx.x, lane = tid & 63, w = tid >> 6, half = lane >> 5, l31 = lane & 31;
    const u32 row0 = blockIdx.y * 256 + w * 64;
    const u32 n_tiles = (n_chunk + 63) / 64, G = gridDim.x;
    u32 t = blockIdx.x;
    if (t >= n_tiles) return;
    if (tid == 0) *stage_cnt = 0;
    i32x4 a[2][KS];
    static_for<0, 2 * KS>([&](auto Ic) __attribute__((always_inline)) {
        constexpr int i = decltype(Ic)::value / KS, s = decltype(Ic)::value % KS;
        const u32 row = row0 + 32 * i + l31;
        const i32x4 v = *(const i32x4 *)(qdig + (u64)(row < B ? row : B - 1) * K + 32 * s + 16 * half);
        a[i][s] = row < B ? v : i32x4{0, 0, 0, 0};
        asm volatile("" : "+a"(a[i][s]));
    });
    float T[2][16];
#pragma unroll
    for (int i = 0; i < 2; i++)
#pragma unroll
        for (int r = 0; r < 16; r++) {
            const u32 row = row0 + 32 * i + (r & 3) + 8 * (r >> 2) + 4 * half, rc = row < B ? row : B - 1;
// ... 474 lines not shown
            static_for<0, KS>([&](auto Sc) __attribute__((always_inline)) {
                constexpr int s = decltype(Sc)::value;
                constexpr bool expand = s < PIECES;
                constexpr int it = ORDER >= 1 ? (s == 2 ? 1 : 0) : (s < PIECES ? s : 0) >> 1, pp = ORDER >= 1 && s == 2 ? 0 : s & 1;
                constexpr bool last_of_slot = ORDER >= 1 ? s >= 1 : pp == 1;
                if (s + 2 < KS) bf[(s + 2) % 3] = *(const i32x4 *)(bt + 32 * (s + 2));
                const i32x4 b = bf[s % 3];
                if constexpr (ORDER >= 2) {
                    const uint4 src = it == 1 ? make_uint4(raw[RS][u][1].x, 0u, raw[RS][u][1].z, 0u) : raw[RS][u][it];
                    u32 o[4] = {0, 0, 0, 0};
                    __builtin_amdgcn_sched_barrier(0);
                    fp4_mfma<s == 0>(acc[0], a[0][s], b);
                    __builtin_amdgcn_sched_barrier(0);
                    if (expand) {
                        o[0] = q2_nibble_dword(src, pp, 0);
                        o[1] = q2_nibble_dword(src, pp, 1);
                    }
                    __builtin_amdgcn_sched_barrier(0);
                    fp4_mfma<s == 0>(acc[1], a[1][s], b);
                    __builtin_amdgcn_sched_barrier(0);
                    if (expand) {
                        o[2] = q2_nibble_dword(src, pp, 2);
                        o[3] = q2_nibble_dword(src, pp, 3);
                        const int j = it == 1 ? xj : w, ppx = it == 1 ? xp : pp;
                        *(uint4 *)(areg_lds + (size_t)(P ^ 1) * TW * LDB + (size_t)(64 * u + lane) * LDB + j * 32 + ppx * 16) = make_uint4(o[0], o[1], o[2], o[3]);
                        if (last_of_slot) load_raw(tt + AHEAD * G, raw[RS][u], u, it);
                    }
                    __builtin_amdgcn_sched_barrier(0);
                } else {
                    fp4_mfma<s == 0>(acc[0], a[0][s], b);
                    fp4_mfma<s == 0>(acc[1], a[1][s], b);
                    if (expand) {
                        store_piece(P ^ 1, raw[RS][u], u, it, pp);
                        if (last_of_slot) load_raw(tt + AHEAD * G, raw[RS][u], u, it);
                    }
                }
            });
            if constexpr (ORDER >= 2) asm volatile("" : "+v"(acc[0]), "+v"(acc[1]));
            const float rx = metric == 0u ? 4.0f * __builtin_amdgcn_rcpf(xm) : 4.0f;
#pragma unroll
            for (int i = 0; i < 2; i++) {
                float best = -__builtin_inff();
#pragma unroll
                for (int r = 0; r < 16; r++) best = fmaxf(best, __builtin_fmaf(acc[i][r], rx, -T[i][r]));
                if (best >= 0.0f && colx < n_chunk) {
                    u32 rbase = row0 + 32 * i + 4 * half;
                    asm volatile("" : "+v"(rbase));
#pragma unroll
                    for (int r = 0; r < 16; r++) {
                        const u32 row = rbase + (r & 3) + 8 * (r >> 2);
                        const float q4 = acc[i][r];
                        if (row < B && __builtin_fmaf(q4, rx, -T[i][r]) >= 0.0f) {
                            const u32 dot = (u32)(q4 * 4.0f);
                            const u32 sp = atomicAdd(stage_cnt, 1u);
                            if (sp < AREG_STAGE) {
                                stage[3 * sp] = colx;
                                stage[3 * sp + 1] = row;
                                stage[3 * sp + 2] = dot;
                            } else
                                areg_append(fo, qmags, mags, metric, n0, colx, row, dot);
                        }
                    }
                }
            }
        });
        __syncthreads();
    };
    while (true) {
        tile_body(std::integral_constant<int, 0>{}, t);
        t += G;
        if (t >= n_tiles) break;
        tile_body(std::integral_constant<int, 1>{}, t);
        t += G;
        if (t >= n_tiles) break;
    }
    const u32 staged = min(*stage_cnt, (u32)AREG_STAGE);
    for (u32 e = tid; e < staged; e += 512) areg_append(fo, qmags, mags, metric, n0, stage[3 * e], stage[3 * e + 1], stage[3 * e + 2]);
}

template <int KC, bool Q2>
__global__ __launch_bounds__(256) void level_table_areg(const uint8_t *__restrict__ qcodes ,
                                                        const u32 *__restrict__ qsums, u32 B, const uint8_t *__restrict__ tcodes,
                                                        const u32 *__restrict__ tcsums, u64 row_stride , u32 ncols,
                                                        float *__restrict__ tab, u64 tab_stride) {
    constexpr int K = KC * 64, KS = KC * 2, LDB = K + 16;
    constexpr int PC = Q2 ? KC : K / 16;
    constexpr int NP = (64 * PC + 255) / 256;
    extern __shared__ __attribute__((aligned(16))) unsigned char areg_lds[];
    const int tid = threadIdx.x, lane = tid & 63, w = tid >> 6, half = lane >> 5, l31 = lane & 31;
    const u32 row0 = blockIdx.y * 256 + w * 64;
    const u32 n_tiles = (ncols + 63) / 64, G = gridDim.x;
    u32 t = blockIdx.x;
    if (t >= n_tiles) return;
    i32x4 a[2][KS];
    static_for<0, 2 * KS>([&](auto Ic) __attribute__((always_inline)) {
        constexpr int i = decltype(Ic)::value / KS, s = decltype(Ic)::value % KS;
        const u32 row = row0 + 32 * i + l31;
        i32x4 v = *(const i32x4 *)(qcodes + (u64)(row < B ? row : B - 1) * K + 32 * s + 16 * half);
        if constexpr (!Q2) v = v ^ (int)0x80808080;
        a[i][s] = row < B ? v : i32x4{0, 0, 0, 0};
        asm volatile("" : "+a"(a[i][s]));
    });
    int rqs[2][16];
#pragma unroll
    for (int i = 0; i < 2; i++)
#pragma unroll
        for (int r = 0; r < 16; r++) {
            const u32 row = row0 + 32 * i + (r & 3) + 8 * (r >> 2) + 4 * half;
            rqs[i][r] = Q2 ? 0 : 128 * (int)qsums[row < B ? row : B - 1] - 16384 * K;
        }
    uint4 raw[NP];
    auto load_tile = [&](u32 tile) __attribute__((always_inline)) {
#pragma unroll
        for (int p = 0; p < NP; p++) {
            const u32 g = (u32)p * 256u + (u32)tid, gg = g < 64u * PC ? g : 0u, c = gg / (u32)PC, pc = gg % (u32)PC;
            const u32 col = tile * 64 + c, cc = col < ncols ? col : ncols - 1;
            raw[p] = *(const uint4 *)(tcodes + (u64)cc * row_stride + (u64)pc * 16);
        }
    };
    auto store_tile = [&](int buf) __attribute__((always_inline)) {
#pragma unroll
        for (int p = 0; p < NP; p++) {
            const u32 g = (u32)p * 256u + (u32)tid, c = g / (u32)PC, pc = g % (u32)PC;
            if (64 * PC % 256 != 0 && g >= 64u * PC) continue;
            unsigned char *dst = areg_lds + (size_t)buf * 64 * LDB + (size_t)c * LDB;
            if constexpr (Q2) {
#pragma unroll
                for (int pp = 0; pp < 4; pp++) *(uint4 *)(dst + (size_t)pc * 64 + pp * 16) = q2_piece_perm(raw[p], pp);
            } else {
                uint4 v = raw[p];
                v.x ^= 0x80808080u; v.y ^= 0x80808080u; v.z ^= 0x80808080u; v.w ^= 0x80808080u;
                *(uint4 *)(dst + (size_t)pc * 16) = v;
            }
        }
    };
    load_tile(t);
    store_tile(0);
    __syncthreads();
    int P = 0;
    while (true) {
        const bool more = t + G < n_tiles;
        if (more) load_tile(t + G);
        const unsigned char *bt = areg_lds + (size_t)P * 64 * LDB + l31 * LDB + 16 * half;
        i32x16 acc[2][2];
        i32x4 bf[3][2];
#pragma unroll
        for (int s = 0; s < 2 && s < KS; s++) {
            bf[s][0] = *(const i32x4 *)(bt + 32 * s);
            bf[s][1] = *(const i32x4 *)(bt + 32 * LDB + 32 * s);
        }
        static_for<0, KS>([&](auto Sc) __attribute__((always_inline)) {
            constexpr int s = decltype(Sc)::value;
            if (s + 2 < KS) {
                bf[(s + 2) % 3][0] = *(const i32x4 *)(bt + 32 * (s + 2));
                bf[(s + 2) % 3][1] = *(const i32x4 *)(bt + 32 * LDB + 32 * (s + 2));
            }
            __builtin_amdgcn_sched_barrier(0);
            const i32x4 b0 = bf[s % 3][0], b1 = bf[s % 3][1];
            areg_mfma<s == 0>(acc[0][0], a[0][s], b0);
            areg_mfma<s == 0>(acc[0][1], a[0][s], b1);
            areg_mfma<s == 0>(acc[1][0], a[1][s], b0);
            areg_mfma<s == 0>(acc[1][1], a[1][s], b1);
            __builtin_amdgcn_sched_barrier(0);
        });
        auto epilogue = [&](auto fullc) __attribute__((always_inline)) {
            constexpr bool FULL = decltype(fullc)::value;
#pragma unroll
            for (int j = 0; j < 2; j++) {
                const u32 col = t * 64 + 32 * j + l31;
                const bool cv = FULL || col < ncols;
                int cs = 0;
                if constexpr (!Q2) cs = 128 * (int)tcsums[cv ? col : ncols - 1];
#pragma unroll
                for (int i = 0; i < 2; i++) {
                    const u32 rbase = row0 + 32 * i + 4 * half;
                    float *out = tab + (u64)rbase * tab_stride + col;
#pragma unroll
                    for (int r = 0; r < 16; r++) {
                        const u32 dr = (r & 3) + 8 * (r >> 2);
                        const u32 dot = (u32)(acc[i][j][r] + rqs[i][r] + cs);
                        if (FULL || (cv && rbase + dr < B)) out[(u64)dr * tab_stride] = (float)dot;
                    }
                }
            }
        };
        if (row0 + 64 <= B && t * 64 + 64 <= ncols) epilogue(std::true_type{});
        else epilogue(std::false_type{});
        if (!more) break;
        store_tile(P ^ 1);
        __syncthreads();
        P ^= 1;
        t += G;
    }
}

template <int KC, int RB >
__global__ __launch_bounds__(256) void flat_scan_u8_areg(const uint8_t *__restrict__ qcodes , const u32 *__restrict__ qsums,
                                                         const float *__restrict__ qmags, u32 B, const uint8_t *__restrict__ codes,
                                                         const u32 *__restrict__ csums, const float *__restrict__ mags, u64 row_stride, u32 n0,
                                                         u32 n_chunk, u32 metric, const FusedOut fo) {
    constexpr int K = KC * 64, KS = KC * 2, LDB = K + 16, PC = K / 16, NP = (64 * PC + 255) / 256;
    extern __shared__ __attribute__((aligned(16))) unsigned char areg_lds[];
    u32 *stage = (u32 *)(areg_lds + (size_t)2 * 64 * LDB), *stage_cnt = stage + 3 * AREG_STAGE;
    const int tid = threadIdx.x, lane = tid & 63, w = tid >> 6, half = lane >> 5, l31 = lane & 31;
    const u32 row0 = blockIdx.y * (128 * RB) + w * (32 * RB);
    const u32 n_tiles = (n_chunk + 63) / 64, G = gridDim.x;
    u32 t = blockIdx.x;
    if (t >= n_tiles) return;
    if (tid == 0) *stage_cnt = 0;
    i32x4 a[RB][KS];
    static_for<0, RB * KS>([&](auto Ic) __attribute__((always_inline)) {
        constexpr int i = decltype(Ic)::value / KS, s = decltype(Ic)::value % KS;
        const u32 row = row0 + 32 * i + l31;
        i32x4 v = *(const i32x4 *)(qcodes + (u64)(row < B ? row : B - 1) * K + 32 * s + 16 * half);
        v = v ^ (int)0x80808080;
        a[i][s] = row < B ? v : i32x4{0, 0, 0, 0};
        asm volatile("" : "+a"(a[i][s]));
    });
    int rqs[RB][16];
    float T[RB][16];
#pragma unroll
    for (int i = 0; i < RB; i++)
#pragma unroll
        for (int r = 0; r < 16; r++) {
            const u32 row = row0 + 32 * i + (r & 3) + 8 * (r >> 2) + 4 * half, rc = row < B ? row : B - 1;
            rqs[i][r] = 128 * (int)qsums[rc] - 16384 * K;
            const u64 k = fo.thr[rc];
            const float qm = qmags[rc];
            const float lo = k == 0ull ? -1.0f : simkey_inv((u32)(k >> 32)) * (1.0f - 4e-6f);
            const float v = metric == 0u ? lo * qm : lo;
            T[i][r] = row < B ? v : __builtin_inff();
        }
    uint4 raw[NP];
    auto load_tile = [&](u32 tile) __attribute__((always_inline)) {
#pragma unroll
        for (int p = 0; p < NP; p++) {
            const u32 g = (u32)p * 256u + (u32)tid, gg = g < 64u * PC ? g : 0u, c = gg / (u32)PC, pc = gg % (u32)PC;
            const u32 col = tile * 64 + c, cc = col < n_chunk ? col : n_chunk - 1;
            raw[p] = *(const uint4 *)(codes + (u64)(n0 + cc) * row_stride + (u64)pc * 16);
        }
    };
    auto store_tile = [&](int buf) __attribute__((always_inline)) {
#pragma unroll
        for (int p = 0; p < NP; p++) {
            const u32 g = (u32)p * 256u + (u32)tid, c = g / (u32)PC, pc = g % (u32)PC;
            if (64 * PC % 256 != 0 && g >= 64u * PC) continue;
            uint4 v = raw[p];
            v.x ^= 0x80808080u; v.y ^= 0x80808080u; v.z ^= 0x80808080u; v.w ^= 0x80808080u;
            *(uint4 *)(areg_lds + (size_t)buf * 64 * LDB + (size_t)c * LDB + (size_t)pc * 16) = v;
        }
    };
    load_tile(t);
    store_tile(0);
    __syncthreads();
    int P = 0;
    while (true) {
        const bool more = t + G < n_tiles;
        if (more) load_tile(t + G);
        const unsigned char *bt = areg_lds + (size_t)P * 64 * LDB + l31 * LDB + 16 * half;
        int csj[2];
        float xmj[2];
#pragma unroll
        for (int j = 0; j < 2; j++) {
            const u32 col = t * 64 + 32 * j + l31, gc = n0 + (col < n_chunk ? col : n_chunk - 1);
            csj[j] = (int)csums[gc];
            xmj[j] = mags[gc];
        }
        i32x16 acc[RB][2];
        i32x4 bf[3][2];
#pragma unroll
        for (int s = 0; s < 2 && s < KS; s++) {
            bf[s][0] = *(const i32x4 *)(bt + 32 * s);
            bf[s][1] = *(const i32x4 *)(bt + 32 * LDB + 32 * s);
        }
        static_for<0, KS>([&](auto Sc) __attribute__((always_inline)) {
// ... 64 lines not shown
}
template <int KC>
static hipError_t launch_areg_kc(dim3 grid, hipStream_t st, const uint8_t *qdig, const float *qmags, u32 B, const uint8_t *codes, const float *mags,
                                 u64 row_stride, u32 n0, u32 nc, u32 metric, const FusedOut &fo) {
    const size_t lds = (size_t)2 * 64 * (KC * 64 + 16) + (size_t)AREG_STAGE * 12 + 16;
    hipError_t e = hipFuncSetAttribute((const void *)flat_scan_q2_areg<KC>, hipFuncAttributeMaxDynamicSharedMemorySize, (int)lds);
    if (e != hipSuccess) return e;
    hipLaunchKernelGGL((flat_scan_q2_areg<KC>), grid, dim3(256), lds, st, qdig, qmags, B, codes, mags, row_stride, n0, nc, metric, fo);
    return hipGetLastError();
}
template <int KC>
static hipError_t launch_fp4_kc(dim3 grid, hipStream_t st, const uint8_t *qnib, const float *qmags, u32 B, const uint8_t *codes, const float *mags,
                                u64 row_stride, u32 n0, u32 nc, u32 metric, const FusedOut &fo) {
    const size_t lds = (size_t)2 * 64 * (KC * 32 + 16) + (size_t)AREG_STAGE * 12 + 16;
    if constexpr (KC == 12) {
        const long long w8 = tune_or(TUNE_FLAT_FP4_W8, 4);
        auto go = [&](auto Oc) -> hipError_t {
            constexpr int ORDER = decltype(Oc)::value, TW = ORDER >= 3 ? 128 : 64;
            const size_t lds8 = (size_t)2 * TW * (KC * 32 + 16) + (size_t)AREG_STAGE * 12 + 16;
            hipError_t e8 = hipFuncSetAttribute((const void *)flat_scan_q2_fp4_w8<KC, ORDER>, hipFuncAttributeMaxDynamicSharedMemorySize, (int)lds8);
            if (e8 != hipSuccess) return e8;
            const dim3 g8(std::min(grid.x, (nc + TW - 1) / TW), grid.y);
            hipLaunchKernelGGL((flat_scan_q2_fp4_w8<KC, ORDER>), g8, dim3(512), lds8, st, qnib, qmags, B, codes, mags, row_stride, n0, nc, metric, fo);
            return hipGetLastError();
        };
        if (w8 == 1) return go(std::integral_constant<int, 0>{});
        if (w8 == 2) return go(std::integral_constant<int, 1>{});
        if (w8 == 3) return go(std::integral_constant<int, 2>{});
        if (w8 >= 4) return go(std::integral_constant<int, 3>{});
    }
    hipError_t e = hipFuncSetAttribute((const void *)flat_scan_q2_fp4<KC>, hipFuncAttributeMaxDynamicSharedMemorySize, (int)lds);
    if (e != hipSuccess) return e;
    hipLaunchKernelGGL((flat_scan_q2_fp4<KC>), grid, dim3(256), lds, st, qnib, qmags, B, codes, mags, row_stride, n0, nc, metric, fo);
    return hipGetLastError();
}
hipError_t launch_flat_scan(u32 kdims, u32 n_cus, hipStream_t st, const uint8_t *qdig, const float *qmags, u32 B, const uint8_t *codes,
                              const float *mags, u64 row_stride, u32 n0, u32 nc, u32 metric, const FusedOut &fo, bool fp4) {
    const u32 n_tiles = (nc + 63) / 64;
    dim3 grid(std::min(n_tiles, n_cus), (B + 255) / 256);
    if (fp4) {
#define FP4_CASE(KC) case KC: return launch_fp4_kc<KC>(grid, st, qdig, qmags, B, codes, mags, row_stride, n0, nc, metric, fo)
        switch (kdims / 64) {
            FP4_CASE(2); FP4_CASE(4); FP4_CASE(6); FP4_CASE(8); FP4_CASE(12); FP4_CASE(16);
            default: return hipErrorInvalidValue;
        }
#undef FP4_CASE
    }
#define AREG_CASE(KC) case KC: return launch_areg_kc<KC>(grid, st, qdig, qmags, B, codes, mags, row_stride, n0, nc, metric, fo)
    switch (kdims / 64) {
        AREG_CASE(2); AREG_CASE(4); AREG_CASE(6); AREG_CASE(8); AREG_CASE(12); AREG_CASE(16);
        default: return hipErrorInvalidValue;
    }
#undef AREG_CASE
}


template <int KC>
static hipError_t launch_u8_kc(u32 n_cus, hipStream_t st, const uint8_t *qcodes, const u32 *qsums, const float *qmags, u32 B, const uint8_t *codes,
                               const u32 *csums, const float *mags, u64 row_stride, u32 n0, u32 nc, u32 metric, const FusedOut &fo) {
    constexpr int RB = KC > 12 ? 1 : 2;
    const size_t lds = (size_t)2 * 64 * (KC * 64 + 16) + (size_t)AREG_STAGE * 12 + 16;
    hipError_t e = hipFuncSetAttribute((const void *)flat_scan_u8_areg<KC, RB>, hipFuncAttributeMaxDynamicSharedMemorySize, (int)lds);
    if (e != hipSuccess) return e;
    const dim3 grid(std::min((nc + 63) / 64, n_cus), (B + 128 * RB - 1) / (128 * RB));
    hipLaunchKernelGGL((flat_scan_u8_areg<KC, RB>), grid, dim3(256), lds, st, qcodes, qsums, qmags, B, codes, csums, mags, row_stride, n0, nc, metric, fo);
    return hipGetLastError();
}
hipError_t launch_flat_scan_u8(u32 kdims, u32 n_cus, hipStream_t st, const uint8_t *qcodes, const u32 *qsums, const float *qmags, u32 B, const uint8_t *codes,
                               const u32 *csums, const float *mags, u64 row_stride, u32 n0, u32 nc, u32 metric, const FusedOut &fo) {
#define U8_CASE(KC) case KC: return launch_u8_kc<KC>(n_cus, st, qcodes, qsums, qmags, B, codes, csums, mags, row_stride, n0, nc, metric, fo)
    switch (kdims / 64) {
        U8_CASE(2); U8_CASE(4); U8_CASE(6); U8_CASE(8); U8_CASE(12); U8_CASE(16);
        default: return hipErrorInvalidValue;
    }
#undef U8_CASE
}

bool level_table_areg_supported(int eng, u64 row_stride) {
    if (eng == ENG_U8) return row_stride % 64 == 0 && flat_scan_supported((u32)row_stride);
    if (eng == ENG_Q2) return row_stride % 16 == 0 && flat_scan_supported((u32)(row_stride / 16) * 64);
    return false;
}
template <int KC, bool Q2>
static hipError_t launch_table_kc(dim3 grid, hipStream_t st, const uint8_t *qcodes, const u32 *qsums, u32 B, const uint8_t *tcodes, const u32 *tcsums,
                                  u64 row_stride, u32 ncols, float *tab, u64 tab_stride) {
    const size_t lds = (size_t)2 * 64 * (KC * 64 + 16);
    hipError_t e = hipFuncSetAttribute((const void *)level_table_areg<KC, Q2>, hipFuncAttributeMaxDynamicSharedMemorySize, (int)lds);
    if (e != hipSuccess) return e;
    hipLaunchKernelGGL((level_table_areg<KC, Q2>), grid, dim3(256), lds, st, qcodes, qsums, B, tcodes, tcsums, row_stride, ncols, tab, tab_stride);
    return hipGetLastError();
}
hipError_t launch_level_table_areg(int eng, u32 n_cus, hipStream_t st, const uint8_t *qcodes, const u32 *qsums, u32 B, const uint8_t *tcodes, const u32 *tcsums,
                                   u64 row_stride, u32 ncols, float *tab, u64 tab_stride) {
    const u32 n_tiles = (ncols + 63) / 64, row_groups = (B + 255) / 256;
    const u32 G = std::max(1u, std::min(n_tiles, n_cus / std::max(1u, std::min(row_groups, n_cus))));
    dim3 grid(G, row_groups);
    const u32 kc = eng == ENG_Q2 ? (u32)(row_stride / 16) : (u32)(row_stride / 64);
#define TAB_CASE(KC)                                                                                                                          \
    case KC:                                                                                                                                  \
        return eng == ENG_Q2 ? launch_table_kc<KC, true>(grid, st, qcodes, qsums, B, tcodes, tcsums, row_stride, ncols, tab, tab_stride)     \
                             : launch_table_kc<KC, false>(grid, st, qcodes, qsums, B, tcodes, tcsums, row_stride, ncols, tab, tab_stride)
    switch (kc) {
        TAB_CASE(2); TAB_CASE(4); TAB_CASE(6); TAB_CASE(8); TAB_CASE(12); TAB_CASE(16);
        default: return hipErrorInvalidValue;
    }
#undef TAB_CASE
}

hipError_t launch_flat_scan_expand_queries(const uint8_t *qcodes, u64 row_stride, u32 B, u32 kdims, uint8_t *digits, hipStream_t st, bool fp4) {
    if (fp4) {
        hipLaunchKernelGGL(expand_q2_nibbles_kernel, dim3((u32)(((u64)B * (kdims / 64) + 255) / 256)), dim3(256), 0, st, qcodes, row_stride, B, kdims, digits);
        return hipGetLastError();
    }
    hipLaunchKernelGGL(expand_q2_digits_perm_kernel, dim3((u32)(((u64)B * (kdims / 64) + 255) / 256)), dim3(256), 0, st, qcodes, row_stride, B, kdims, digits);
    return hipGetLastError();
}

}
```

cosdata_amd/csrc/kernels_walk.hip:

```cpp
#include <hip/hip_runtime.h>

#include <algorithm>
#include <cstdlib>

#include "engine_types.h"
#include "tuning.h"
#include "walk_common.h"
#include "walk_plan.h"

using namespace cosdev;

namespace {

template <int ENG>
__global__ __launch_bounds__(256) void quantize_rows_kernel(const float *__restrict__ x, u64 x_stride, u32 n, u32 dim, float lo,
                                                            float hi, uint8_t *__restrict__ codes, u64 row_stride,
                                                            float *__restrict__ mags, float *__restrict__ raw_mags) {
    const int lane = threadIdx.x & 63;
    const u32 row = blockIdx.x * (blockDim.x >> 6) + (threadIdx.x >> 6);
    if (row >= n) return;
    const float *xr = x + (u64)row * x_stride;
    uint8_t *cr = codes + (u64)row * row_stride;
    float rn = 0.0f;
    const bool need_seq = (raw_mags != nullptr) || (ENG != ENG_U8);
    if (need_seq) rn = seq_norm_wave(xr, dim, lane);
    if (raw_mags && lane == 0) raw_mags[row] = rn;
    if constexpr (ENG == ENG_U8) {
        u32 ss = 0;
        for (u32 i = lane; i < (u32)row_stride; i += 64) {
            uint8_t q = 0;
            if (i < dim) {
                float c = rust_min(rust_max(xr[i], lo), hi);
                float v = __fmul_rn(__fdiv_rn(__fsub_rn(c, lo), __fsub_rn(hi, lo)), 255.0f);
                q = rust_f32_as_u8(v);
            }
            cr[i] = q;
            ss += (u32)q * (u32)q;
        }
#pragma unroll
        for (int m = 32; m > 0; m >>= 1) ss += (u32)__shfl_xor((int)ss, m, 64);
        if (lane == 0) mags[row] = sqrtf((float)ss);
    } else if constexpr (ENG == ENG_Q2) {
        const u32 nch = (u32)(row_stride / 16);
        for (u32 c = 0; c < nch; c++) {
            u32 i = c * 64 + lane;
            u32 lvl = 0;
            if (i < dim) lvl = rust_f32_as_usize_low2(floorf(__fdiv_rn(__fadd_rn(xr[i], 1.0f), 0.5f)));
            u64 p0 = __ballot((lvl >> 1) & 1u);
            u64 p1 = __ballot(lvl & 1u);
            if (lane == 0) {
                *(u64 *)(cr + (u64)c * 16) = p0;
                *(u64 *)(cr + (u64)c * 16 + 8) = p1;
            }
        }
        if (lane == 0) mags[row] = rn;
    } else if constexpr (ENG == ENG_Q1) {
        const u32 nch = (u32)(row_stride / 16);
        for (u32 c = 0; c < 2 * nch; c++) {
            const u32 i = c * 64 + lane;
            u32 lvl = 0;
            if (i < dim) lvl = rust_f32_as_usize_low(floorf(__fdiv_rn(__fadd_rn(xr[i], 1.0f), 1.0f)), 1u);
            const u64 p0 = __ballot(lvl & 1u);
            if (lane == 0) *(u64 *)(cr + (u64)c * 8) = p0;
        }
        if (lane == 0) mags[row] = rn;
    } else if constexpr (ENG == ENG_Q3) {
        const u32 nch = (u32)(row_stride / 16);
        for (u32 c = 0; c < nch; c += 2) {
            const u32 i = c * 32 + lane;
            u32 lvl = 0;
            if (i < dim) lvl = rust_f32_as_usize_low(floorf(__fdiv_rn(__fadd_rn(xr[i], 1.0f), 0.25f)), 7u);
            const u64 p0 = __ballot((lvl >> 2) & 1u), p1 = __ballot((lvl >> 1) & 1u), p2 = __ballot(lvl & 1u);
            if (lane == 0) {
                *(uint4 *)(cr + (u64)c * 16) = make_uint4((u32)p0, (u32)p1, (u32)p2, 0u);
                if (c + 1 < nch) *(uint4 *)(cr + (u64)(c + 1) * 16) = make_uint4((u32)(p0 >> 32), (u32)(p1 >> 32), (u32)(p2 >> 32), 0u);
            }
        }
        if (lane == 0) mags[row] = rn;
    } else if constexpr (ENG == ENG_F16) {
        __half *ch = (__half *)cr;
        for (u32 i = lane; i < (u32)(row_stride / 2); i += 64) ch[i] = i < dim ? __float2half_rn(xr[i]) : __float2half_rn(0.0f);
        if (lane == 0) mags[row] = rn;
    } else {
        float *cf = (float *)cr;
        for (u32 i = lane; i < (u32)(row_stride / 4); i += 64) cf[i] = i < dim ? xr[i] : 0.0f;
        if (lane == 0) mags[row] = rn;
    }
}

#include "walk_kernel.inc"

struct FinalizeArgs {
    const float *queries;
    u64 q_stride;
    const float *q_raw_mags;
    const u32 *walk_ids;
    const float *walk_sims;
    const u32 *walk_counts;
    const int32_t *walk_status;
    u32 B, top_k;
    u32 *out_ids;
    float *out_scores;
    u32 *out_counts;
    int32_t *out_status;
    u64 *out_rerank_rows;
    const u32 *q_order;
    u32 *slow_list;
    u32 *slow_count;
};

template <int NWV>
__device__ __forceinline__ void finalize_sync() {
    if constexpr (NWV > 1) __syncthreads();
    else { __builtin_amdgcn_s_waitcnt(0); __builtin_amdgcn_wave_barrier(); }
}
template <int NWV>
__device__ __forceinline__ void rerank_wide(const IndexDev &ix, const float *qf, const u32 *cand, u32 ncand, float mag_query, u64 *keys, int lane, int wave) {
    for (u32 base = (u32)wave * 8u; base < ncand; base += 8u * (u32)NWV) {
        const u32 my = base + (u32)(lane >> 3);
        const u32 id = my < ncand ? cand[my] : 0u;
        const u32 rrow = id / ix.id_stride;
        const float dp = f32_oct_dot(ix.raw + (u64)rrow * ix.raw_stride, qf, ix.dim, lane & 7);
        const float cs = x86_div(dp, __fmul_rn(mag_query, ix.raw_mags[rrow]));
        if ((lane & 7) == 0 && my < ncand) keys[my] = pack_key(simkey(cs), id);
// ... 248 lines not shown
            const u64 key = pack_key(metric_key(metric, smv[u]), id);
            const u64 keep = ballot64((u32)lane < cc[u] && !drop && key >= T);
            const u32 nk = (u32)__popcll(keep);
            if (n + nk > (u32)FAST_CAP) { overflow = true; break; }
            if (__builtin_amdgcn_inverse_ballot_w64(keep)) surv[n + (u32)__popcll(keep & ((1ull << lane) - 1ull))] = key;
            n += nk;
        }
        if (overflow) break;
    }
    if (overflow) {
        if (lane == 0) fa.slow_list[atomicAdd(fa.slow_count, 1u)] = qi;
        if constexpr (NWV > 1) {
            if (lane == 0) cand[64] = 0xFFFFFFFFu;
            __syncthreads();
            __syncthreads();
        }
        return;
    }
    __builtin_amdgcn_s_waitcnt(0);
    __builtin_amdgcn_wave_barrier();
    u64 k[2];
#pragma unroll
    for (int r = 0; r < 2; r++) {
        const u32 e = (u32)lane * 2u + (u32)r;
        k[r] = e < n ? surv[e] : 0ull;
    }
    bitonic_sort_desc<2>(k, lane);
    const u64 prev_last = shfl_up1_u64(k[1]);
    const bool keep0 = k[0] != 0ull && (lane == 0 || k[0] != prev_last), keep1 = k[1] != 0ull && k[1] != k[0];
    const u32 mine = (keep0 ? 1u : 0u) + (keep1 ? 1u : 0u);
    u32 incl = mine;
#pragma unroll
    for (int d = 1; d < 64; d <<= 1) {
        const u32 t = (u32)__shfl_up((int)incl, d, 64);
        if (lane >= d) incl += t;
    }
    u32 pos = incl - mine;
    const u32 total = readlane_u32(incl, 63);
    const u32 ncand = total < want ? total : want;
    if (keep0) { if (pos < ncand) cand[pos] = (u32)k[0]; pos++; }
    if (keep1) { if (pos < ncand) cand[pos] = (u32)k[1]; }
    const u32 nout = ncand < fa.top_k ? ncand : fa.top_k;
    u64 res[1] = {0ull};
    if constexpr (NWV > 1) {
        if (lane == 0) cand[64] = ncand;
        __syncthreads();
        rerank_wide<NWV>(ix, qf, cand, ncand, mag_query, surv, lane, 0);
        __syncthreads();
        res[0] = (u32)lane < ncand ? surv[lane] : 0ull;
    } else {
    __builtin_amdgcn_s_waitcnt(0);
    __builtin_amdgcn_wave_barrier();

    const int pair = lane >> 1;
    for (u32 base = 0; base < ncand; base += 32) {
        const u32 my = base + (u32)pair;
        const u32 id = my < ncand ? cand[my] : 0u;
        const u32 rrow = id / ix.id_stride;
        const float dp = f32_pair_dot(ix.raw + (u64)rrow * ix.raw_stride, qf, ix.dim, lane & 1);
        const float cs = x86_div(dp, __fmul_rn(mag_query, ix.raw_mags[rrow]));
        const u64 key = my < ncand ? pack_key(simkey(cs), id) : 0ull;
        const int from = (2 * (lane - (int)base)) & 63;
        const u32 klo = (u32)__shfl((int)(u32)key, from, 64), khi = (u32)__shfl((int)(u32)(key >> 32), from, 64);
        if ((u32)lane >= base && (u32)lane < base + 32) res[0] = ((u64)khi << 32) | klo;
    }
    }
    bitonic_sort_desc<1>(res, lane);
    if ((u32)lane < nout) {
        fa.out_ids[(u64)qi * fa.top_k + lane] = (u32)res[0] + ix.id_base;
        fa.out_scores[(u64)qi * fa.top_k + lane] = simkey_inv((u32)(res[0] >> 32));
    }
    if (lane == 0) {
        fa.out_counts[qi] = nout;
        fa.out_status[qi] = COS_OK;
        if (fa.out_rerank_rows) fa.out_rerank_rows[qi] = ncand;
    }
}

}

namespace cosdev {

hipError_t launch_quantize_rows(int eng, const float *x, u64 x_stride, u32 n, u32 dim, float lo, float hi, uint8_t *codes,
                                u64 row_stride, float *mags, float *raw_mags, hipStream_t st) {
    if (n == 0) return hipSuccess;
    dim3 block(256), grid((n + 3) / 4);
    switch (eng) {
    case ENG_U8: hipLaunchKernelGGL(quantize_rows_kernel<ENG_U8>, grid, block, 0, st, x, x_stride, n, dim, lo, hi, codes, row_stride, mags, raw_mags); break;
    case ENG_Q2: hipLaunchKernelGGL(quantize_rows_kernel<ENG_Q2>, grid, block, 0, st, x, x_stride, n, dim, lo, hi, codes, row_stride, mags, raw_mags); break;
    case ENG_F32: hipLaunchKernelGGL(quantize_rows_kernel<ENG_F32>, grid, block, 0, st, x, x_stride, n, dim, lo, hi, codes, row_stride, mags, raw_mags); break;
    case ENG_F16: hipLaunchKernelGGL(quantize_rows_kernel<ENG_F16>, grid, block, 0, st, x, x_stride, n, dim, lo, hi, codes, row_stride, mags, raw_mags); break;
    case ENG_Q1: hipLaunchKernelGGL(quantize_rows_kernel<ENG_Q1>, grid, block, 0, st, x, x_stride, n, dim, lo, hi, codes, row_stride, mags, raw_mags); break;
    case ENG_Q3: hipLaunchKernelGGL(quantize_rows_kernel<ENG_Q3>, grid, block, 0, st, x, x_stride, n, dim, lo, hi, codes, row_stride, mags, raw_mags); break;
    default: return hipErrorInvalidValue;
    }
    return hipGetLastError();
}

size_t walk_smem_bytes(const IndexDev &ix, u32 ef, int eng, u32 mmax, u32 win_bytes) {
    size_t b = (size_t)mmax * 8 + (size_t)ef * 8 + 64 * 4 * 2 + (size_t)win_bytes;
    b = (b + 15) & ~(size_t)15;
    if (eng == ENG_F32) b += (size_t)ix.row_stride;
    if (eng == ENG_F16) b += ((size_t)ix.dim * 4 + 15) & ~(size_t)15;
    return b + 16;
}

static int walk_pb_policy(u32 B, u32 ef, bool upper_range_of_a_split_walk) {
    const int forced = (int)tune_or(TUNE_WALK_PB, 0), forced_upper = (int)tune_or(TUNE_WALK_PB_UPPER, 0);
    if (upper_range_of_a_split_walk && (forced_upper == 4 || forced_upper == 8)) return forced_upper;
    if (forced == 4 || forced == 8) return forced;
    if (upper_range_of_a_split_walk && ef > 64u) return 4;
    return ef > 256u ? 4 : 8;
}

static u32 walk_merge_min_policy(u32 ef) {
    const long long forced = tune_or(TUNE_WALK_MERGE_MIN, -1);
    if (forced >= 0) return (u32)std::min<long long>(forced, 65);
    return ef <= 64u ? 4u : 3u;
}

template <int ENG, int CH, bool G64>
static hipError_t launch_walk_r(const IndexDev &ix, const WalkArgs &wa_in, hipStream_t st) {
    WalkArgs wa = wa_in;
    wa.merge_min = wa.tab != nullptr ? walk_merge_min_policy(wa.ef) : 0u;
    const u32 lf = wa.phase ? wa.level_first : ix.num_layers, ll = wa.phase ? wa.level_last : 0u;
    u32 mmax = 1;
    for (u32 l = ll; l <= lf; l++) mmax = std::max(mmax, ix.lv[l].M);
    constexpr bool TABLE_ENG = ENG == ENG_U8 || ENG == ENG_Q2;
    const bool all_tab = TABLE_ENG && wa.tab != nullptr && ll >= wa.tab_level_min && tune_or(TUNE_WALK_UPPER_LDS_PAD, 0) >= 0;
    wa.smem_mmax = mmax;
    size_t pad = 0;
    if (wa.phase != 0u && wa.level_last >= 1u) pad = (size_t)std::max<long long>(0, std::min<long long>(tune_or(TUNE_WALK_UPPER_LDS_PAD, 0), 48 << 10));
    dim3 grid(wa.B), block(64);
    const bool exact = ix.visited_mode != 0;
    constexpr bool HAS_PB8 = ENG == ENG_U8 && G64 && CH == 1;
    const bool pb8 = HAS_PB8 && walk_pb_policy(wa.B, wa.ef, wa.phase != 0u && wa.level_last >= 1u) == 8;
#define WALK(R_)                                                                                                          \
    do {                                                                                                                  \
        wa.smem_win_bytes = (all_tab && (R_) <= 4) ? (u32)(((64 * (R_) + 1) * 8 + 15) & ~15) : (u32)(LA * 64 * 4 * 3);         \
        const size_t smem = walk_smem_bytes(ix, wa.ef, ENG, mmax, wa.smem_win_bytes) + pad;                                \
        if constexpr (HAS_PB8) {                                                                                          \
            if (pb8) {                                                                                                    \
                if (exact) hipLaunchKernelGGL((walk_kernel<ENG, CH, R_, G64, true, 8>), grid, block, smem, st, ix, wa);   \
                else hipLaunchKernelGGL((walk_kernel<ENG, CH, R_, G64, false, 8>), grid, block, smem, st, ix, wa);        \
                break;                                                                                                    \
            }                                                                                                             \
        }                                                                                                                 \
        if (exact) hipLaunchKernelGGL((walk_kernel<ENG, CH, R_, G64, true>), grid, block, smem, st, ix, wa);              \
        else hipLaunchKernelGGL((walk_kernel<ENG, CH, R_, G64, false>), grid, block, smem, st, ix, wa);                   \
    } while (0)
    if (wa.ef <= 64) WALK(1);
    else if (wa.ef <= 128 && tune_or(TUNE_WALK_R2, 1) != 0) WALK(2);
    else if (wa.ef <= 256) WALK(4);
    else if (wa.ef <= 512) WALK(8);
    else if (wa.ef <= 1024) WALK(16);
    else return hipErrorInvalidValue;
#undef WALK
    return hipGetLastError();
}

hipError_t launch_walk_lat(int eng, const IndexDev &ix, const WalkArgs &wa, hipStream_t st);
hipError_t launch_walk_lat4(int eng, const IndexDev &ix, const WalkArgs &wa, hipStream_t st);
hipError_t launch_walk_general(int eng, const IndexDev &ix, const WalkArgs &wa, hipStream_t st);

hipError_t launch_walk(int eng, const IndexDev &ix, const WalkArgs &wa, WalkKernel kernel, hipStream_t st) {
    if (wa.B == 0) return hipSuccess;
    if (kernel == WalkKernel::General) return launch_walk_general(eng, ix, wa, st);
    if (kernel == WalkKernel::Lat4) return launch_walk_lat4(eng, ix, wa, st);
    if (kernel == WalkKernel::Lat1) return launch_walk_lat(eng, ix, wa, st);
    const u32 ch = (eng == ENG_F32 || eng == ENG_F16) ? 1 : (ix.nchunks + ix.G - 1) / ix.G;
    switch (eng) {
    case ENG_U8:
        if (ch == 1) return ix.G == 64 ? launch_walk_r<ENG_U8, 1, true>(ix, wa, st) : launch_walk_r<ENG_U8, 1, false>(ix, wa, st);
        if (ch == 2) return launch_walk_r<ENG_U8, 2, true>(ix, wa, st);
        if (ch == 3) return launch_walk_r<ENG_U8, 3, true>(ix, wa, st);
        if (ch == 4) return launch_walk_r<ENG_U8, 4, true>(ix, wa, st);
// ... 61 lines not shown
```

cosdata_amd/csrc/tuning.h:

```cpp
#pragma once
#include <cstdint>

namespace cosdev {

enum TuneKey : int {
    TUNE_WALK_CHAIN_MIN_B,
    TUNE_WALK_ORDER_MIN_B,
    TUNE_WALK_SIDE_MIN_B,
    TUNE_WALK_SPLIT_LEVELS,
    TUNE_WALK_TABLE_COLS,
    TUNE_WALK_TABLE_MIN_B,
    TUNE_WALK_TABLE_MAX_BYTES,
    TUNE_WALK_TABLE_GEMM,
    TUNE_HOST_PIPELINE_MIN_B,
    TUNE_FLAT_UNFUSED,
    TUNE_FLAT_TILE_KERNEL,
    TUNE_FLAT_PF,
    TUNE_FLAT_FP4,
    TUNE_BM25_BLOCKS,
    TUNE_SPARSE_LAYOUT,
    TUNE_WALK_PB,
    TUNE_WALK_PB_UPPER,
    TUNE_WALK_LAT,
    TUNE_WALK_LAT4,
    TUNE_WALK_SMALL_TABLE_TK,
    TUNE_WALK_LAT_WARM,
    TUNE_WALK_LAT_LA,
    TUNE_WALK_LAT4_E,
    TUNE_FINALIZE_FAST,
    TUNE_SHARDSET_FORCE_RCCL,
    TUNE_BUILD_PROFILE,
    TUNE_WALK_MERGE_MIN,
    TUNE_WALK_ADJ_MAG,
    TUNE_WALK_TABLE_RULE_C,
    TUNE_WALK_TABLE_AFTER_SORT,
    TUNE_WALK_UPPER_LDS_PAD,
    TUNE_WALK_R2,
    TUNE_FINALIZE_WIDE_MAX_B,
    TUNE_FLAT_FP4_W8,
    TUNE_COUNT
};

constexpr long long TUNE_UNSET = INT64_MIN;

long long tune(TuneKey k);
inline long long tune_or(TuneKey k, long long dflt) {
    const long long v = tune(k);
    return v == TUNE_UNSET ? dflt : v;
}

}
```

cosdata_amd/csrc/tuning.hip:

```cpp
#include <atomic>
#include <cstdlib>
#include <cstring>
#include <mutex>

#include "engine_internal.h"
#include "tuning.h"

namespace cosdev {
namespace {

const char *const NAMES[TUNE_COUNT] = {
    "walk_chain_min_b", "walk_order_min_b", "walk_side_min_b", "walk_split_levels", "walk_table_cols", "walk_table_min_b",
    "walk_table_max_bytes", "walk_table_gemm", "host_pipeline_min_b", "flat_unfused", "flat_tile_kernel", "flat_pf", "flat_fp4",
    "bm25_blocks", "sparse_layout", "walk_pb", "walk_pb_upper", "walk_lat", "walk_lat4", "walk_small_table_tk", "walk_lat_warm",
    "walk_lat_la", "walk_lat4_e", "finalize_fast", "shardset_force_rccl", "build_profile",
    "walk_merge_min", "walk_adj_mag", "walk_table_rule_c", "walk_table_after_sort", "walk_upper_lds_pad", "walk_r2", "finalize_wide_max_b", "flat_fp4_w8",
};
std::atomic<long long> g_values[TUNE_COUNT];
std::once_flag g_once;

int find_key(const char *name, size_t len) {
    for (int k = 0; k < TUNE_COUNT; k++)
        if (strlen(NAMES[k]) == len && strncmp(NAMES[k], name, len) == 0) return k;
    return -1;
}

void init_once() {
    std::call_once(g_once, [] {
        for (auto &v : g_values) v.store(TUNE_UNSET, std::memory_order_relaxed);
        const char *e = getenv("COS_TUNING");
        while (e && *e) {
            const char *end = strchr(e, ',');
            const size_t item = end ? (size_t)(end - e) : strlen(e);
            const char *eq = (const char *)memchr(e, '=', item);
            if (eq) {
                const int k = find_key(e, (size_t)(eq - e));
                char *stop = nullptr;
                const long long v = strtoll(eq + 1, &stop, 10);
                if (k >= 0 && stop != eq + 1) g_values[k].store(v, std::memory_order_relaxed);
            }
            e = end ? end + 1 : nullptr;
        }
    });
}

}

long long tune(TuneKey k) {
    init_once();
    return g_values[k].load(std::memory_order_relaxed);
}

}

using namespace cosdev;

extern "C" int32_t cos_tuning_set(const char *name, int64_t value) {
    if (!name) return cos_fail(COS_ERR_INVALID, "null knob name");
    const int k = find_key(name, strlen(name));
    if (k < 0) return cos_fail(COS_ERR_INVALID, "unknown tuning knob '%s'", name);
    if (value == TUNE_UNSET) return cos_fail(COS_ERR_INVALID, "INT64_MIN is the 'unset' marker: use cos_tuning_clear");
    init_once();
    g_values[k].store(value, std::memory_order_relaxed);
    return COS_OK;
}

extern "C" int32_t cos_tuning_clear(const char *name) {
    init_once();
    if (!name) {
        for (auto &v : g_values) v.store(TUNE_UNSET, std::memory_order_relaxed);
        return COS_OK;
    }
    const int k = find_key(name, strlen(name));
    if (k < 0) return cos_fail(COS_ERR_INVALID, "unknown tuning knob '%s'", name);
    g_values[k].store(TUNE_UNSET, std::memory_order_relaxed);
    return COS_OK;
}

extern "C" int32_t cos_tuning_get(const char *name, int64_t *out_value, int32_t *out_is_set) {
    if (!name || !out_value || !out_is_set) return cos_fail(COS_ERR_INVALID, "null argument");
    const int k = find_key(name, strlen(name));
    if (k < 0) return cos_fail(COS_ERR_INVALID, "unknown tuning knob '%s'", name);
    const long long v = tune((TuneKey)k);
    *out_is_set = v != TUNE_UNSET;
    *out_value = v == TUNE_UNSET ? 0 : v;
    return COS_OK;
}
```

cosdata_amd/csrc/walk_plan.h:

```cpp
#pragma once
#include <algorithm>
#include <cstdint>

namespace cosdev {

constexpr int WALK_PLAN_MAX_LEVELS = 16;
constexpr int WALK_PLAN_ENG_U8 = 0, WALK_PLAN_ENG_Q2 = 1;
constexpr uint32_t WALK_PLAN_FAST_MAX_EF = 1024u;

constexpr uint32_t ADJ_MAG_REFILL_MIN_B = 1024u, ADJ_MAG_USE_MIN_B = 4096u;

enum class WalkKernel : uint8_t {
    General,
    Throughput,
    Lat1,
    Lat4
};

struct WalkPlanIn {
    int eng;
    uint32_t storage;
    uint32_t nchunks, G;
    uint32_t num_layers, M[WALK_PLAN_MAX_LEVELS], shortlist, visited_mode, mdim;
    uint32_t B, ef;
    bool chain;
    bool no_self_seed;
    uint32_t lat_max_B, lat4_max_B;
    bool small_table_tk;
    uint32_t adj_mag_mode;
    uint32_t table_min_B;
    uint32_t order_min_B, chain_min_B, side_min_B;
    long long table_after_sort;
    bool table_supported;
    bool adj_mag_valid;
};

struct WalkHave {
    uint32_t table_level_min, table_cols;
    bool table_buffer;
    uint32_t n_order_keys, order_level0;
    bool order_buffers;
};

struct WalkPlan {
    WalkKernel kernel;
    bool ordered;
    bool use_table;
    bool table_waits_for_sort;
    uint32_t use_adj_mag;
    bool refill_adj_mag;
    bool chained;
    bool side_stream;
    bool prepare_order, prepare_table;
    uint32_t table_level_min, table_cols, cut_after_level;
};

inline bool walk_rows_over_64_slots(const WalkPlanIn &in) {
    for (uint32_t l = 0; l <= in.num_layers; l++)
        if (std::min(in.M[l], in.shortlist) > 64u) return true;
    return false;
}

inline bool walk_general_needed(const WalkPlanIn &in) {
    if (in.ef > WALK_PLAN_FAST_MAX_EF) return true;
    if (in.nchunks != 0u && in.G != 0u && (in.nchunks + in.G - 1u) / in.G > (in.storage == 0u  ? 4u : 1u)) return true;
    return walk_rows_over_64_slots(in);
}

inline bool walk_latency_domain(const WalkPlanIn &in, uint32_t max_B) {
    if (max_B == 0 || in.B > max_B) return false;
    if (in.visited_mode != 0) return false;
    if (in.eng != WALK_PLAN_ENG_U8 && in.eng != WALK_PLAN_ENG_Q2) return false;
    if (in.nchunks == 0 || in.nchunks > 64u) return false;
    if (in.ef == 0 || in.ef > 256) return false;
    return true;
}

inline WalkKernel walk_fast_kernel(const WalkPlanIn &in, bool table_available) {
    if (in.no_self_seed) return WalkKernel::Throughput;
    const bool lat4 = walk_latency_domain(in, in.lat4_max_B) && std::max(in.M[0], in.M[in.num_layers]) <= 64u;
    if (table_available && in.small_table_tk && in.eng == WALK_PLAN_ENG_U8)
        return in.ef > 128u && lat4 ? WalkKernel::Lat4 : WalkKernel::Throughput;
    if (lat4) return WalkKernel::Lat4;
    if (walk_latency_domain(in, in.lat_max_B)) return WalkKernel::Lat1;
    return WalkKernel::Throughput;
}

inline WalkPlan walk_plan(const WalkPlanIn &in, const WalkHave *have = nullptr) {
    WalkPlan p{};
    const bool general = walk_general_needed(in);
    p.ordered = !general && in.order_min_B && in.B >= in.order_min_B && in.ef <= 256u && (!have || (have->n_order_keys > 0 && have->order_buffers));
    bool table = !general && in.table_min_B && (have ? have->table_level_min != 0 && have->table_buffer : in.table_supported);
    const bool table_size = in.B >= in.table_min_B || in.B <= in.lat4_max_B;
    if (general) p.kernel = WalkKernel::General;
    else if (p.ordered) {
        p.kernel = WalkKernel::Throughput;
        table = table && table_size;
    } else {
        const WalkKernel with_table = walk_fast_kernel(in, true);
        table = table && ((with_table == WalkKernel::Lat4 && in.eng == WALK_PLAN_ENG_U8) || (with_table == WalkKernel::Throughput && table_size));
        p.kernel = table ? with_table : walk_fast_kernel(in, false);
    }
    p.use_table = table;
    p.chained = in.chain && in.B >= in.chain_min_B;
    if (have && table) {
        p.table_level_min = have->table_level_min;
        p.table_cols = have->table_cols;
        p.table_waits_for_sort = p.chained && (in.table_after_sort == 2 || (in.table_after_sort == 1 && (uint64_t)have->table_cols * in.B >= (1ull << 30)));
    }
    if (have && p.ordered) p.cut_after_level = have->order_level0;
    if (in.adj_mag_valid && in.adj_mag_mode != 0)
        for (uint32_t l = 0; l <= in.num_layers; l++)
            if (in.adj_mag_mode == 2 || (in.ef <= 2u * in.M[l] && in.B >= ADJ_MAG_USE_MIN_B)) p.use_adj_mag |= 1u << l;
    p.refill_adj_mag = !in.adj_mag_valid && in.B >= ADJ_MAG_REFILL_MIN_B;
    p.side_stream = in.side_min_B && in.B >= in.side_min_B;
    p.prepare_order = p.ordered;
    p.prepare_table = p.use_table;
    return p;
}

}
```

include/cosdata_hip.h:

```cpp
#ifndef COSDATA_HIP_H
#define COSDATA_HIP_H

#include <stddef.h>
#include <stdint.h>

#ifdef __cplusplus
extern "C" {
#endif

#define COS_ABI_VERSION 1u

typedef enum { COS_METRIC_COSINE = 0, COS_METRIC_EUCLIDEAN = 1, COS_METRIC_HAMMING = 2, COS_METRIC_DOT = 3 } cos_metric;
typedef enum { COS_STORAGE_U8 = 0, COS_STORAGE_SUBBYTE = 1, COS_STORAGE_F16 = 2, COS_STORAGE_F32 = 3 } cos_storage;

typedef enum {
    COS_OK = 0,
    COS_ERR_STORAGE_MISMATCH = 1,
    COS_ERR_CALCULATION = 2,
    COS_ERR_INVALID = 3,
    COS_ERR_UNIMPLEMENTED = 4,
    COS_ERR_HIP = 5,
    COS_ERR_NOT_READY = 6,
    COS_ERR_NO_DEVICE = 7
} cos_status;
// ... 29 lines not shown
    uint64_t seed;
} cos_params;

typedef struct cos_index cos_index;

typedef struct {
    uint64_t evals;
    uint64_t expansions;
    uint64_t adj_bytes;
    uint64_t rerank_rows;
    float walk_ms;
    float finalize_ms;
    float prep_ms;
    uint32_t reserved;
} cos_search_stats;

int32_t cos_index_create(const cos_params *params, cos_index **out);
int32_t cos_index_destroy(cos_index *ix);
const char *cos_last_error_string(void);
int32_t cos_device_count(int32_t *out);
int32_t cos_hbm_probe(int32_t device, uint32_t kind, uint64_t buffer_bytes, uint32_t row_bytes, uint32_t iters,
                      double *out_gbps);

int32_t cos_index_upload_vectors(cos_index *ix, const float *raw, uint32_t n, uint32_t flags);
int32_t cos_index_set_root(cos_index *ix, const float *root_raw);
int32_t cos_index_upload_graph_level(cos_index *ix, uint32_t level, uint32_t n_nodes, const uint32_t *node_ids,
                                     const uint32_t *nbr_ids);
int32_t cos_index_level_count(const cos_index *ix, uint32_t level, uint32_t *n_nodes);
int32_t cos_index_download_graph_level(const cos_index *ix, uint32_t level, uint32_t *node_ids, uint32_t *nbr_ids);
int32_t cos_index_download_codes(const cos_index *ix, void *codes, float *mags);
int32_t cos_index_download_root(const cos_index *ix, float *root_raw);

#define COS_LOAD_DEFAULT 0u
#define COS_LOAD_VERIFY_CODES 1u
int32_t cos_index_load_reference_dir(cos_index *ix, const char *dense_hnsw_dir, uint32_t root_ptr_offset, uint32_t flags);
int32_t cos_reference_dir_level_counts(const char *dense_hnsw_dir, uint32_t num_layers, uint32_t neighbors_count,
                                       uint32_t level0_neighbors_count, uint32_t *level_counts );
int32_t cos_reference_dir_read_level(const char *dense_hnsw_dir, uint32_t num_layers, uint32_t neighbors_count,
                                     uint32_t level0_neighbors_count, uint32_t level, uint32_t *node_ids, uint32_t *nbr_ids);

int32_t cos_index_build(cos_index *ix, uint32_t batch_size);
int32_t cos_index_append(cos_index *ix, const float *raw, uint32_t m, uint32_t flags, uint32_t batch_size );
int32_t cos_index_delete(cos_index *ix, const uint32_t *ids, uint32_t m);
int32_t cos_index_restore_link_state(cos_index *ix);
int32_t cos_index_release_link_state(cos_index *ix);

int32_t cos_search_batch(cos_index *ix, const float *queries, uint32_t B, uint32_t top_k, uint32_t *out_ids,
                         float *out_scores, uint32_t *out_counts, int32_t *out_status);
int32_t cos_search_batch_device(cos_index *ix, const float *d_queries, uint32_t B, uint32_t top_k, uint32_t *d_out_ids,
                                float *d_out_scores, uint32_t *d_out_counts, int32_t *d_out_status, void *stream);
int32_t cos_ann_search_batch(cos_index *ix, const float *queries, uint32_t B, uint32_t *out_ids, float *out_sims,
                             uint32_t *out_counts, int32_t *out_status);
int32_t cos_index_set_coalescing(cos_index *ix, uint32_t max_queries, uint32_t window_us);
typedef struct cos_coalescing_stats {
    uint64_t launches;
    uint64_t queries;
    uint64_t requests;
    uint64_t closed_full;
    uint64_t closed_quiet;
    uint64_t closed_deadline;
    uint64_t solo_calls;
} cos_coalescing_stats;
int32_t cos_index_coalescing_stats(cos_index *ix, cos_coalescing_stats *out);
int32_t cos_index_set_ef_search(cos_index *ix, uint32_t ef_search);
int32_t cos_index_set_visited_mode(cos_index *ix, uint32_t mode);
#define COS_LATENCY_MODE_DEFAULT_MAX_B 2048u
int32_t cos_index_set_latency_mode(cos_index *ix, uint32_t max_queries);
#define COS_LATENCY_WAVES_DEFAULT_MAX_B 512u
int32_t cos_index_set_latency_waves(cos_index *ix, uint32_t max_queries);
#define COS_WALK_ORDER_DEFAULT_MIN_B 8192u
int32_t cos_index_set_walk_order(cos_index *ix, uint32_t min_queries);
int32_t cos_index_walk_order_cuts(cos_index *ix, uint32_t *out_levels, uint32_t cap, uint32_t *out_n);
#define COS_WALK_TABLE_DEFAULT_MIN_B 1u
#define COS_WALK_TABLE_DEFAULT_MAX_COLS 8192u
#define COS_WALK_TABLE_AUTO 0xFFFFFFFFu
int32_t cos_index_set_walk_table(cos_index *ix, uint32_t max_cols, uint32_t min_queries);
int32_t cos_index_walk_table_info(cos_index *ix, uint32_t *out_level_min, uint32_t *out_cols);
typedef struct {
    uint32_t struct_size;
    uint32_t queries;
    uint32_t table_level_min;
    uint32_t table_cols;
    uint32_t cut_after_level;
    uint32_t reserved;
    float table_ms;
    float upper_ms, sort_ms, lower_ms;
    double table_int8_ops;
    uint64_t table_evals;
    uint64_t upper_evals, upper_expansions, upper_adj_bytes;
    uint64_t lower_evals, lower_expansions, lower_adj_bytes;
} cos_walk_split;
int32_t cos_index_last_walk_split(cos_index *ix, void *stream, cos_walk_split *out);
int32_t cos_index_enable_timing(cos_index *ix, int32_t on);
int32_t cos_index_last_stats(cos_index *ix, void *stream, cos_search_stats *out);
typedef struct {
    uint32_t launches;
    float prep_ms_sum, walk_ms_sum, finalize_ms_sum;
    float walk_ms_min, walk_ms_max;
} cos_timing_summary;
int32_t cos_index_timing_summary(cos_index *ix, void *stream, cos_timing_summary *out);

int32_t cos_index_enable_metadata(cos_index *ix, uint32_t mdim , uint32_t max_replicas_per_node);
int32_t cos_index_upload_meta_nodes(cos_index *ix, uint32_t n_nodes, const uint32_t *node_ids, const int32_t *mbits);
int32_t cos_index_upload_meta_graph_level(cos_index *ix, uint32_t level, uint32_t n_nodes, const uint32_t *node_ids,
                                          const uint32_t *nbr_ids);
int32_t cos_index_build_meta(cos_index *ix, uint32_t n_nodes, const uint32_t *node_ids, const int32_t *mbits, const uint8_t *max_levels,
                             uint32_t batch_size );
int32_t cos_index_meta_level_count(cos_index *ix, uint32_t level, uint32_t *out);
int32_t cos_index_download_meta_graph_level(cos_index *ix, uint32_t level, uint32_t *node_ids, uint32_t *nbr_ids);
int32_t cos_search_filtered_batch(cos_index *ix, const float *queries, uint32_t B, const uint32_t *filter_offsets,
                                  const int8_t *filter_dims, uint32_t top_k, uint32_t *out_ids, float *out_scores,
                                  uint32_t *out_counts, int32_t *out_status);
int32_t cos_ann_search_filtered_batch(cos_index *ix, const float *queries, uint32_t B, const uint32_t *filter_offsets,
                                      const int8_t *filter_dims, uint32_t *out_ids, float *out_sims, uint32_t *out_counts,
                                      int32_t *out_status);

int32_t cos_quantize_batch(uint32_t storage, uint32_t resolution, uint32_t dim, float range_lo, float range_hi,
                           const float *x, uint32_t n, void *codes, float *mags);
size_t cos_code_bytes(uint32_t storage, uint32_t resolution, uint32_t dim);
int32_t cos_sample_values_range(const float *x, uint32_t n, uint32_t dim, float clamp_margin_percent, float *range_lo,
                                float *range_hi);
int32_t cos_distance_batch(uint32_t metric, uint32_t storage, uint32_t resolution, uint32_t dim, const void *x_codes,
                           const float *x_mags, uint32_t nx, const void *y_codes, const float *y_mags, uint32_t ny,
                           const uint32_t *pair_x, const uint32_t *pair_y, uint32_t n_pairs, float *out,
                           int32_t *status);
int32_t cos_bruteforce_topk(cos_index *ix, const float *queries, uint32_t B, uint32_t k, uint32_t *out_ids,
                            float *out_scores);

typedef struct {
    float gemm_ms;
    uint32_t gemm_launches;
    double int8_ops;
    double code_bytes;
} cos_flat_stats;
int32_t cos_flat_search_batch(cos_index *ix, const float *queries, uint32_t B, uint32_t top_k, uint32_t *out_ids,
                              float *out_scores, uint32_t *out_counts, cos_flat_stats *stats );

typedef struct cos_bm25 cos_bm25;
int32_t cos_bm25_create(int32_t device, const uint32_t *term_hashes, const uint64_t *offsets, uint32_t n_terms,
                        const uint32_t *doc_ids, const float *tfs, uint32_t documents_count, cos_bm25 **out);
int32_t cos_bm25_destroy(cos_bm25 *b);
int32_t cos_bm25_insert(cos_bm25 *b, const uint32_t *doc_ids, const uint64_t *doc_offsets, uint32_t m, const uint32_t *term_hashes,
                        const float *tfs);
int32_t cos_bm25_delete(cos_bm25 *b, const uint32_t *doc_ids, const uint64_t *doc_offsets, uint32_t m, const uint32_t *term_hashes);
typedef struct {
    uint32_t struct_size;
    uint32_t documents_count;
    uint32_t n_terms;
    uint32_t largest_doc_id;
    uint32_t dir_rows;
    uint32_t dir_tiles;
    uint32_t reserved;
    uint64_t postings;
    uint64_t tombstones;
    uint64_t device_bytes;
} cos_bm25_index_stats;
int32_t cos_bm25_stats(cos_bm25 *b, cos_bm25_index_stats *out);
int32_t cos_bm25_download(cos_bm25 *b, uint32_t *n_terms, uint64_t *n_postings, uint32_t *term_hashes, uint64_t *offsets,
                          uint32_t *doc_ids, float *tfs, uint8_t *tombstones);
int32_t cos_bm25_search_batch(cos_bm25 *b, const uint32_t *q_terms, const uint32_t *q_offsets, uint32_t B,
                              uint32_t top_k, uint32_t *out_ids, float *out_scores, uint32_t *out_counts);
int32_t cos_bm25_search_batch_device(cos_bm25 *b, const uint32_t *q_terms, const uint32_t *q_offsets, uint32_t B, uint32_t top_k,
                                     uint32_t *d_out_ids, float *d_out_scores, uint32_t *d_out_counts, void *stream);
int32_t cos_rrf_fuse_batch(const uint32_t *dense_ids, const uint32_t *dense_counts, uint32_t dense_stride,
                           const uint32_t *sparse_ids, const uint32_t *sparse_counts, uint32_t sparse_stride, uint32_t B,
                           float fusion_constant_k, uint32_t top_k, uint32_t *out_ids, float *out_scores,
                           uint32_t *out_counts);
// ... 90 lines not shown
```

Baseline: 1.021 million.

## Split level-table GEMM into early and late phases via a shared work queue

Reworks the level-table GEMM kernel into a persistent, queue-driven form in which workgroups pull stripes of tiles from an atomic counter. A configurable number of early workgroups can start once the previous batch's upper walk finishes, and the remaining work runs after that batch's walk completes, so the table build overlaps the chained walk. The u8 code sums are now computed inside the quantize kernel instead of in a separate launch. The early-workgroup default is 0, so by default only the queue-based scheduling and the fused sums are active; the kernel and event logic become more complex.

```diff
diff --git a/cosdata_amd/_lib.py b/cosdata_amd/_lib.py
--- a/cosdata_amd/_lib.py
+++ b/cosdata_amd/_lib.py
@@ -44,7 +44,7 @@
 class CosWalkSplit(C.Structure):
     _fields_ = [
         ("struct_size", C.c_uint32), ("queries", C.c_uint32), ("table_level_min", C.c_uint32), ("table_cols", C.c_uint32),
-        ("cut_after_level", C.c_uint32), ("reserved", C.c_uint32),
+        ("cut_after_level", C.c_uint32), ("table_early_wgs", C.c_uint32),
         ("table_ms", C.c_float), ("upper_ms", C.c_float), ("sort_ms", C.c_float), ("lower_ms", C.c_float),
         ("table_int8_ops", C.c_double), ("table_evals", C.c_uint64),
         ("upper_evals", C.c_uint64), ("upper_expansions", C.c_uint64), ("upper_adj_bytes", C.c_uint64),
diff --git a/cosdata_amd/csrc/engine.hip b/cosdata_amd/csrc/engine.hip
--- a/cosdata_amd/csrc/engine.hip
+++ b/cosdata_amd/csrc/engine.hip
@@ -678,6 +678,7 @@
     const long long env = cosdev::tune_or(cosdev::TUNE_WALK_TABLE_MIN_B, -1);
     return env >= 0 ? (u32)std::min<long long>(env, 0xFFFFFFFFll) : ix->walk_table_min_B;
 }
+static constexpr long long WALK_TABLE_EARLY_WGS_DEFAULT = 0;
 cosdev::WalkPlanIn cos_walk_plan_in(const cos_index *ix, u32 B, u32 ef) {
     cosdev::WalkPlanIn in{};
     in.eng = ix->eng;
@@ -704,6 +705,9 @@
     in.table_after_sort = cosdev::tune_or(cosdev::TUNE_WALK_TABLE_AFTER_SORT, 1);
     in.table_supported = cosdev::level_table_eng_supported(ix->eng, ix->row_stride);
     in.adj_mag_valid = ix->adj_mag_valid;
+    in.table_early_wgs = (u32)std::min<long long>(std::max<long long>(cosdev::tune_or(cosdev::TUNE_WALK_TABLE_EARLY_WGS, WALK_TABLE_EARLY_WGS_DEFAULT), 0), 0xFFFFFFFFll);
+    in.table_queue = cosdev::level_table_gemm_queue(ix->eng, ix->row_stride);
+    in.n_cus = ix->n_cus;
     return in;
 }
 static int32_t ensure_level_table(cos_index *ix) {
@@ -890,6 +894,7 @@
         HIP_TRY(w->stats.alloc((size_t)cap * 4));
         HIP_TRY(w->stats2.alloc((size_t)cap * 4));
         HIP_TRY(w->qsums.alloc(cap));
+        HIP_TRY(w->tab_queue.alloc(16));
         if (ix->eng == ENG_Q2) HIP_TRY(w->qdig.alloc((size_t)cap * (ix->row_stride / 16) * 64));
         HIP_TRY(w->fin_flags.alloc((size_t)cap + 1));
         HIP_TRY(w->rerank_rows.alloc(cap));
@@ -967,6 +972,7 @@
     if (!w->walk_done) HIP_TRY(hipEventCreateWithFlags(&w->walk_done, hipEventDisableTiming));
     if (!w->walk_fin) HIP_TRY(hipEventCreateWithFlags(&w->walk_fin, hipEventDisableTiming));
     if (!w->last_range) HIP_TRY(hipEventCreateWithFlags(&w->last_range, hipEventDisableTiming));
+    if (!w->upper_done) HIP_TRY(hipEventCreateWithFlags(&w->upper_done, hipEventDisableTiming));
     *out = w;
     return COS_OK;
 }
@@ -990,16 +996,25 @@
     hipEvent_t *ev = &w->ev[(size_t)(w->ev_count % Workspace::EV_RING) * Workspace::EV_PER];
     if (timed) HIP_TRY(hipEventRecord(ev[0], st));
     HIP_TRY(launch_quantize_rows(ix->eng, d_queries, ix->p.dim, B, ix->p.dim, ix->p.range_lo, ix->p.range_hi, w->q_codes, ix->row_stride,
-                                 w->q_mags, w->q_raw_mags, st));
+                                 w->q_mags, w->q_raw_mags, st, plan.use_table && ix->eng == ENG_U8 ? w->qsums.p : nullptr));
     if (plan.use_table) {
-        if (plan.table_waits_for_sort) {
-            std::lock_guard<std::mutex> g(ix->chain_mu);
-            if (ix->chain_last_range_ev && ix->chain_last_range_ev != w->last_range) HIP_TRY(hipStreamWaitEvent(st, ix->chain_last_range_ev, 0));
-        }
-        if (timed) HIP_TRY(hipEventRecord(ev[4], st));
-        HIP_TRY(cosdev::launch_level_table(ix->eng, w->q_codes, w->q_mags, w->qsums, w->qdig, B, L.tcodes, L.tmags, L.tcsums, ix->row_stride, plan.table_cols,
-                                           w->tab, L.tab_stride, ix->n_cus, st));
-        if (timed) HIP_TRY(hipEventRecord(ev[5], st));
+        auto table_part = [&](hipEvent_t cos_index::*handle_ev, hipEvent_t own_ev, hipEvent_t *marks, u32 wgs, bool first) -> int32_t {
+            if (plan.table_waits_for_sort) {
+                std::lock_guard<std::mutex> g(ix->chain_mu);
+                if (ix->*handle_ev && ix->*handle_ev != own_ev) HIP_TRY(hipStreamWaitEvent(st, ix->*handle_ev, 0));
+            }
+            if (timed) HIP_TRY(hipEventRecord(marks[0], st));
+            HIP_TRY(cosdev::launch_level_table(ix->eng, w->q_codes, w->q_mags, w->qsums, w->qdig, B, L.tcodes, L.tmags, L.tcsums, ix->row_stride, plan.table_cols,
+                                               w->tab, L.tab_stride, ix->n_cus, st, w->tab_queue, wgs, first, plan.table_waits_for_sort));
+            if (timed) HIP_TRY(hipEventRecord(marks[1], st));
+            return COS_OK;
+        };
+        if (cosdev::level_table_gemm_queue(ix->eng, ix->row_stride)) HIP_TRY(hipMemsetAsync(w->tab_queue, 0, sizeof(u32), st));
+        if (plan.table_early_wgs) {
+            if (int32_t rc = table_part(&cos_index::chain_upper_ev, w->upper_done, ev + 4, plan.table_early_wgs, true)) return rc;
+            if (int32_t rc = table_part(&cos_index::chain_ev, w->walk_done, ev + 8, 0u, false)) return rc;
+        } else if (int32_t rc = table_part(&cos_index::chain_last_range_ev, w->last_range, ev + 4, 0u, true))
+            return rc;
     }
     if (timed) HIP_TRY(hipEventRecord(ev[1], st));
     wa.qcodes = w->q_codes;
@@ -1035,6 +1050,7 @@
     }
     auto walk = [&](hipStream_t s) -> int32_t {
         if (!ordered) {
+            if (chained) HIP_TRY(hipEventRecord(w->upper_done, s));
             if (chained) HIP_TRY(hipEventRecord(w->last_range, s));
             HIP_TRY(launch_walk(ix->eng, dev, wa, plan.kernel, s));
             return COS_OK;
@@ -1053,6 +1069,7 @@
             if (last && chained) HIP_TRY(hipEventRecord(w->last_range, s));
             HIP_TRY(launch_walk(ix->eng, dev, wa, plan.kernel, s));
             if (last) break;
+            if (chained && i == 0) HIP_TRY(hipEventRecord(w->upper_done, s));
             if (timed && i == 0) HIP_TRY(hipEventRecord(ev[6], s));
             HIP_TRY(cosdev::launch_walk_order(w->order, B, L.key_n[i], ix->num_xcd, s));
             if (timed && i == 0) HIP_TRY(hipEventRecord(ev[7], s));
@@ -1069,6 +1086,7 @@
         HIP_TRY(hipEventRecord(w->walk_done, sw));
         ix->chain_ev = w->walk_done;
         ix->chain_last_range_ev = w->last_range;
+        ix->chain_upper_ev = w->upper_done;
     } else {
         if (timed && sw != st) HIP_TRY(hipEventRecord(ev[1], sw));
         if (int32_t rc = walk(sw)) return rc;
@@ -1537,10 +1555,16 @@
     out->table_level_min = plan.table_level_min;
     out->table_cols = plan.table_cols;
     out->cut_after_level = plan.cut_after_level;
+    out->table_early_wgs = plan.use_table ? plan.table_early_wgs : 0u;
     if (w->timed && w->ev_count) {
         hipEvent_t *ev = &w->ev[(size_t)((w->ev_count - 1) % Workspace::EV_RING) * Workspace::EV_PER];
         HIP_TRY(hipEventSynchronize(ev[3]));
         if (plan.use_table) HIP_TRY(hipEventElapsedTime(&out->table_ms, ev[4], ev[5]));
+        if (plan.use_table && plan.table_early_wgs) {
+            float late_ms = 0.f;
+            HIP_TRY(hipEventElapsedTime(&late_ms, ev[8], ev[9]));
+            out->table_ms += late_ms;
+        }
         if (plan.ordered) {
             HIP_TRY(hipEventElapsedTime(&out->upper_ms, ev[1], ev[6]));
             HIP_TRY(hipEventElapsedTime(&out->sort_ms, ev[6], ev[7]));
diff --git a/cosdata_amd/csrc/engine_internal.h b/cosdata_amd/csrc/engine_internal.h
--- a/cosdata_amd/csrc/engine_internal.h
+++ b/cosdata_amd/csrc/engine_internal.h
@@ -31,7 +31,7 @@
 hipError_t launch_link_round(const LinkArgs &a, u32 maxM, const u32 *pend, const u32 *pcount, u32 *next, u32 *next_count, u32 *evq, u32 *evq_count,
                              u32 count_ub, u32 round, hipStream_t st);
 hipError_t launch_quantize_rows(int eng, const float *x, u64 x_stride, u32 n, u32 dim, float lo, float hi, uint8_t *codes,
-                                u64 row_stride, float *mags, float *raw_mags, hipStream_t st);
+                                u64 row_stride, float *mags, float *raw_mags, hipStream_t st, u32 *code_sums = nullptr);
 hipError_t launch_walk(int eng, const IndexDev &ix, const WalkArgs &wa, WalkKernel kernel, hipStream_t st);
 static_assert(WALK_PLAN_MAX_LEVELS == MAX_LEVELS && WALK_PLAN_ENG_U8 == ENG_U8 && WALK_PLAN_ENG_Q2 == ENG_Q2 && WALK_PLAN_FAST_MAX_EF == WALK_FAST_MAX_EF &&
               COS_STORAGE_U8 == 0u && COS_VISITED_REF == 0u, "walk_plan.h restates these");
@@ -54,8 +54,9 @@
 hipError_t launch_level_table_gather(const uint8_t *codes, const float *mags, u64 row_stride, const u32 *node_vec, u32 n, u32 col0,
                                      uint8_t *tcodes, float *tmags, hipStream_t st);
 hipError_t launch_code_sums(const uint8_t *codes, u64 row_stride, u32 n, u32 *sums, hipStream_t st);
-hipError_t launch_level_table(int eng, const uint8_t *qcodes, const float *qmags, u32 *qsums, uint8_t *qdig, u32 B, const uint8_t *tcodes, const float *tmags,
-                              const u32 *tcsums, u64 row_stride, u32 ncols, float *tab, u64 tab_stride, u32 n_cus, hipStream_t st);
+hipError_t launch_level_table(int eng, const uint8_t *qcodes, const float *qmags, const u32 *qsums, uint8_t *qdig, u32 B, const uint8_t *tcodes, const float *tmags,
+                              const u32 *tcsums, u64 row_stride, u32 ncols, float *tab, u64 tab_stride, u32 n_cus, hipStream_t st, u32 *queue, u32 wgs, bool first, bool shared);
+bool level_table_gemm_queue(int eng, u64 row_stride);
 bool level_table_eng_supported(int eng, u64 row_stride);
 int32_t quantize_ref_layout(uint32_t storage, uint32_t res, uint32_t dim, const float *x, uint32_t n, void *codes, float *mags);
 int32_t distance_ref_layout(uint32_t metric, uint32_t storage, uint32_t res, uint32_t dim, const void *x_codes, const float *x_mags, uint32_t nx,
@@ -120,6 +121,7 @@
     DevArr<u64> stats2;
     DevArr<float> tab;
     DevArr<u32> qsums;
+    DevArr<u32> tab_queue;
     DevArr<uint8_t> qdig;
     DevArr<u32> fin_flags;
     DevArr<u64> rerank_rows;
@@ -131,11 +133,12 @@
     DevArr<int32_t> d_out_status;
     DevArr<u32> f_buf;
     static constexpr u32 EV_RING = 128;
-    static constexpr u32 EV_PER = 8;
+    static constexpr u32 EV_PER = 10;
     std::vector<hipEvent_t> ev;
     u32 ev_count = 0;
     hipEvent_t walk_done = nullptr;
     hipEvent_t last_range = nullptr;
+    hipEvent_t upper_done = nullptr;
     hipStream_t walk_stream = nullptr;
     hipEvent_t prep_done = nullptr, walk_fin = nullptr;
     u32 lastB = 0;
@@ -144,7 +147,7 @@
     Workspace() = default;
     Workspace(const Workspace &) = delete;
     ~Workspace() {
-        for (hipEvent_t e : {walk_done, walk_fin, last_range, prep_done}) if (e) (void)hipEventDestroy(e);
+        for (hipEvent_t e : {walk_done, walk_fin, last_range, upper_done, prep_done}) if (e) (void)hipEventDestroy(e);
         for (hipEvent_t e : ev) if (e) (void)hipEventDestroy(e);
         if (walk_stream) (void)hipStreamDestroy(walk_stream);
     }
@@ -213,6 +216,7 @@
     std::mutex chain_mu;
     hipEvent_t chain_ev = nullptr;
     hipEvent_t chain_last_range_ev = nullptr;
+    hipEvent_t chain_upper_ev = nullptr;
     u32 chain_min_B = 16384;
     u32 walk_order_min_B = COS_WALK_ORDER_DEFAULT_MIN_B;
     u32 n_cus = 256;
diff --git a/cosdata_amd/csrc/flat_scan.h b/cosdata_amd/csrc/flat_scan.h
--- a/cosdata_amd/csrc/flat_scan.h
+++ b/cosdata_amd/csrc/flat_scan.h
@@ -39,6 +39,6 @@
 
 bool level_table_areg_supported(int eng, u64 row_stride);
 hipError_t launch_level_table_areg(int eng, u32 n_cus, hipStream_t st, const uint8_t *qcodes, const u32 *qsums, u32 B, const uint8_t *tcodes,
-                                   const u32 *tcsums, u64 row_stride, u32 ncols, float *tab, u64 tab_stride);
+                                   const u32 *tcsums, u64 row_stride, u32 ncols, float *tab, u64 tab_stride, u32 *queue, u32 wgs, bool shared);
 
 }
diff --git a/cosdata_amd/csrc/kernels_flat.hip b/cosdata_amd/csrc/kernels_flat.hip
--- a/cosdata_amd/csrc/kernels_flat.hip
+++ b/cosdata_amd/csrc/kernels_flat.hip
@@ -878,30 +878,30 @@
     return eng == ENG_U8 || (eng == ENG_Q2 && level_table_areg_supported(ENG_Q2, row_stride));
 }
 
-hipError_t launch_level_table(int eng, const uint8_t *qcodes, const float *qmags, u32 *qsums , uint8_t *qdig ,
+bool level_table_gemm_queue(int eng, u64 row_stride) { return level_table_areg_supported(eng, row_stride) && tune_or(TUNE_WALK_TABLE_GEMM, 1) != 0; }
+hipError_t launch_level_table(int eng, const uint8_t *qcodes, const float *qmags, const u32 *qsums , uint8_t *qdig ,
                               u32 B, const uint8_t *tcodes, const float *tmags, const u32 *tcsums, u64 row_stride, u32 ncols, float *tab, u64 tab_stride,
-                              u32 n_cus, hipStream_t st) {
+                              u32 n_cus, hipStream_t st, u32 *queue, u32 wgs, bool first, bool shared) {
     if (B == 0 || ncols == 0) return hipSuccess;
     const bool q2 = eng == ENG_Q2;
     const u32 kdims = q2 ? (u32)(row_stride / 16) * 64 : (u32)((row_stride + 63) / 64 * 64);
     hipError_t e = hipSuccess;
-    if (!q2) e = launch_code_sums(qcodes, row_stride, B, qsums, st);
-    if (e != hipSuccess) return e;
-    if (level_table_areg_supported(eng, row_stride) && tune_or(TUNE_WALK_TABLE_GEMM, 1) != 0) {
-        if (q2) {
+    if (level_table_gemm_queue(eng, row_stride)) {
+        if (q2 && first) {
             e = launch_flat_scan_expand_queries(qcodes, row_stride, B, kdims, qdig, st, false);
             if (e != hipSuccess) return e;
         }
-        return launch_level_table_areg(eng, n_cus ? n_cus : 256u, st, q2 ? qdig : qcodes, (const u32 *)qsums, B, tcodes, tcsums, row_stride, ncols, tab, tab_stride);
-    }
+        return launch_level_table_areg(eng, n_cus ? n_cus : 256u, st, q2 ? qdig : qcodes, qsums, B, tcodes, tcsums, row_stride, ncols, tab, tab_stride, queue, wgs, shared);
+    }
+    if (!first) return hipSuccess;
     const u32 metric = 1u;
     dim3 grid((ncols + CN - 1) / CN, (B + CM - 1) / CM);
     FusedOut fo{nullptr, nullptr, nullptr, 0u, nullptr};
     if (q2)
-        hipLaunchKernelGGL((flat_codes_gemm_i8<ENG_Q2, false, 2>), grid, dim3(512), 0, st, qcodes, qmags, (const u32 *)qsums, B, tcodes, tmags, tcsums, row_stride, 0u,
+        hipLaunchKernelGGL((flat_codes_gemm_i8<ENG_Q2, false, 2>), grid, dim3(512), 0, st, qcodes, qmags, qsums, B, tcodes, tmags, tcsums, row_stride, 0u,
                            ncols, kdims, metric, tab, tab_stride, fo);
     else
-        hipLaunchKernelGGL((flat_codes_gemm_i8<ENG_U8, false, 2>), grid, dim3(512), 0, st, qcodes, qmags, (const u32 *)qsums, B, tcodes, tmags, tcsums, row_stride, 0u,
+        hipLaunchKernelGGL((flat_codes_gemm_i8<ENG_U8, false, 2>), grid, dim3(512), 0, st, qcodes, qmags, qsums, B, tcodes, tmags, tcsums, row_stride, 0u,
                            ncols, kdims, metric, tab, tab_stride, fo);
     return hipGetLastError();
 }
diff --git a/cosdata_amd/csrc/kernels_scan.hip b/cosdata_amd/csrc/kernels_scan.hip
--- a/cosdata_amd/csrc/kernels_scan.hip
+++ b/cosdata_amd/csrc/kernels_scan.hip
@@ -7,6 +7,7 @@
 #include "device_common.h"
 #include "flat_scan.h"
 #include "tuning.h"
+#include "walk_plan.h"
 
 using namespace cosdev;
 
@@ -647,33 +648,34 @@
 __global__ __launch_bounds__(256) void level_table_areg(const uint8_t *__restrict__ qcodes ,
                                                         const u32 *__restrict__ qsums, u32 B, const uint8_t *__restrict__ tcodes,
                                                         const u32 *__restrict__ tcsums, u64 row_stride , u32 ncols,
-                                                        float *__restrict__ tab, u64 tab_stride) {
+                                                        float *__restrict__ tab, u64 tab_stride, u32 *__restrict__ queue, u32 stripe) {
     constexpr int K = KC * 64, KS = KC * 2, LDB = K + 16;
     constexpr int PC = Q2 ? KC : K / 16;
     constexpr int NP = (64 * PC + 255) / 256;
     extern __shared__ __attribute__((aligned(16))) unsigned char areg_lds[];
+    __shared__ u32 s_item;
     const int tid = threadIdx.x, lane = tid & 63, w = tid >> 6, half = lane >> 5, l31 = lane & 31;
-    const u32 row0 = blockIdx.y * 256 + w * 64;
-    const u32 n_tiles = (ncols + 63) / 64, G = gridDim.x;
-    u32 t = blockIdx.x;
-    if (t >= n_tiles) return;
+    const u32 n_tiles = (ncols + 63) / 64, row_groups = (B + 255) / 256, n_items = (n_tiles + stripe - 1) / stripe * row_groups;
+    u32 row0 = 0, rg_now = 0xFFFFFFFFu, t = 0, t_end = 0;
     i32x4 a[2][KS];
-    static_for<0, 2 * KS>([&](auto Ic) __attribute__((always_inline)) {
-        constexpr int i = decltype(Ic)::value / KS, s = decltype(Ic)::value % KS;
-        const u32 row = row0 + 32 * i + l31;
-        i32x4 v = *(const i32x4 *)(qcodes + (u64)(row < B ? row : B - 1) * K + 32 * s + 16 * half);
-        if constexpr (!Q2) v = v ^ (int)0x80808080;
-        a[i][s] = row < B ? v : i32x4{0, 0, 0, 0};
-        asm volatile("" : "+a"(a[i][s]));
-    });
     int rqs[2][16];
-#pragma unroll
-    for (int i = 0; i < 2; i++)
-#pragma unroll
-        for (int r = 0; r < 16; r++) {
-            const u32 row = row0 + 32 * i + (r & 3) + 8 * (r >> 2) + 4 * half;
-            rqs[i][r] = Q2 ? 0 : 128 * (int)qsums[row < B ? row : B - 1] - 16384 * K;
-        }
+    auto load_rows = [&]() __attribute__((always_inline)) {
+        static_for<0, 2 * KS>([&](auto Ic) __attribute__((always_inline)) {
+            constexpr int i = decltype(Ic)::value / KS, s = decltype(Ic)::value % KS;
+            const u32 row = row0 + 32 * i + l31;
+            i32x4 v = *(const i32x4 *)(qcodes + (u64)(row < B ? row : B - 1) * K + 32 * s + 16 * half);
+            if constexpr (!Q2) v = v ^ (int)0x80808080;
+            a[i][s] = row < B ? v : i32x4{0, 0, 0, 0};
+            asm volatile("" : "+a"(a[i][s]));
+        });
+#pragma unroll
+        for (int i = 0; i < 2; i++)
+#pragma unroll
+            for (int r = 0; r < 16; r++) {
+                const u32 row = row0 + 32 * i + (r & 3) + 8 * (r >> 2) + 4 * half;
+                rqs[i][r] = Q2 ? 0 : 128 * (int)qsums[row < B ? row : B - 1] - 16384 * K;
+            }
+    };
     uint4 raw[NP];
     auto load_tile = [&](u32 tile) __attribute__((always_inline)) {
 #pragma unroll
@@ -699,63 +701,78 @@
             }
         }
     };
-    load_tile(t);
-    store_tile(0);
-    __syncthreads();
-    int P = 0;
     while (true) {
-        const bool more = t + G < n_tiles;
-        if (more) load_tile(t + G);
-        const unsigned char *bt = areg_lds + (size_t)P * 64 * LDB + l31 * LDB + 16 * half;
-        i32x16 acc[2][2];
-        i32x4 bf[3][2];
-#pragma unroll
-        for (int s = 0; s < 2 && s < KS; s++) {
-            bf[s][0] = *(const i32x4 *)(bt + 32 * s);
-            bf[s][1] = *(const i32x4 *)(bt + 32 * LDB + 32 * s);
-        }
-        static_for<0, KS>([&](auto Sc) __attribute__((always_inline)) {
-            constexpr int s = decltype(Sc)::value;
-            if (s + 2 < KS) {
-                bf[(s + 2) % 3][0] = *(const i32x4 *)(bt + 32 * (s + 2));
-                bf[(s + 2) % 3][1] = *(const i32x4 *)(bt + 32 * LDB + 32 * (s + 2));
-            }
-            __builtin_amdgcn_sched_barrier(0);
-            const i32x4 b0 = bf[s % 3][0], b1 = bf[s % 3][1];
-            areg_mfma<s == 0>(acc[0][0], a[0][s], b0);
-            areg_mfma<s == 0>(acc[0][1], a[0][s], b1);
-            areg_mfma<s == 0>(acc[1][0], a[1][s], b0);
-            areg_mfma<s == 0>(acc[1][1], a[1][s], b1);
-            __builtin_amdgcn_sched_barrier(0);
-        });
-        auto epilogue = [&](auto fullc) __attribute__((always_inline)) {
-            constexpr bool FULL = decltype(fullc)::value;
-#pragma unroll
-            for (int j = 0; j < 2; j++) {
-                const u32 col = t * 64 + 32 * j + l31;
-                const bool cv = FULL || col < ncols;
-                int cs = 0;
-                if constexpr (!Q2) cs = 128 * (int)tcsums[cv ? col : ncols - 1];
-#pragma unroll
-                for (int i = 0; i < 2; i++) {
-                    const u32 rbase = row0 + 32 * i + 4 * half;
-                    float *out = tab + (u64)rbase * tab_stride + col;
-#pragma unroll
-                    for (int r = 0; r < 16; r++) {
-                        const u32 dr = (r & 3) + 8 * (r >> 2);
-                        const u32 dot = (u32)(acc[i][j][r] + rqs[i][r] + cs);
-                        if (FULL || (cv && rbase + dr < B)) out[(u64)dr * tab_stride] = (float)dot;
+        __syncthreads();
+        if (tid == 0) s_item = atomicAdd(queue, 1u);
+        __syncthreads();
+        const u32 item = s_item;
+        if (item >= n_items) break;
+        const u32 rg = item % row_groups;
+        t = item / row_groups * stripe;
+        t_end = min(n_tiles, t + stripe);
+        if (rg != rg_now) {
+            rg_now = rg;
+            row0 = rg * 256 + w * 64;
+            load_rows();
+        }
+        load_tile(t);
+        store_tile(0);
+        __syncthreads();
+        int P = 0;
+        while (true) {
+            const bool more = t + 1 < t_end;
+            if (more) load_tile(t + 1);
+            const unsigned char *bt = areg_lds + (size_t)P * 64 * LDB + l31 * LDB + 16 * half;
+            i32x16 acc[2][2];
+            i32x4 bf[3][2];
+#pragma unroll
+            for (int s = 0; s < 2 && s < KS; s++) {
+                bf[s][0] = *(const i32x4 *)(bt + 32 * s);
+                bf[s][1] = *(const i32x4 *)(bt + 32 * LDB + 32 * s);
+            }
+            static_for<0, KS>([&](auto Sc) __attribute__((always_inline)) {
+                constexpr int s = decltype(Sc)::value;
+                if (s + 2 < KS) {
+                    bf[(s + 2) % 3][0] = *(const i32x4 *)(bt + 32 * (s + 2));
+                    bf[(s + 2) % 3][1] = *(const i32x4 *)(bt + 32 * LDB + 32 * (s + 2));
+                }
+                __builtin_amdgcn_sched_barrier(0);
+                const i32x4 b0 = bf[s % 3][0], b1 = bf[s % 3][1];
+                areg_mfma<s == 0>(acc[0][0], a[0][s], b0);
+                areg_mfma<s == 0>(acc[0][1], a[0][s], b1);
+                areg_mfma<s == 0>(acc[1][0], a[1][s], b0);
+                areg_mfma<s == 0>(acc[1][1], a[1][s], b1);
+                __builtin_amdgcn_sched_barrier(0);
+            });
+            auto epilogue = [&](auto fullc) __attribute__((always_inline)) {
+                constexpr bool FULL = decltype(fullc)::value;
+#pragma unroll
+                for (int j = 0; j < 2; j++) {
+                    const u32 col = t * 64 + 32 * j + l31;
+                    const bool cv = FULL || col < ncols;
+                    int cs = 0;
+                    if constexpr (!Q2) cs = 128 * (int)tcsums[cv ? col : ncols - 1];
+#pragma unroll
+                    for (int i = 0; i < 2; i++) {
+                        const u32 rbase = row0 + 32 * i + 4 * half;
+                        float *out = tab + (u64)rbase * tab_stride + col;
+#pragma unroll
+                        for (int r = 0; r < 16; r++) {
+                            const u32 dr = (r & 3) + 8 * (r >> 2);
+                            const u32 dot = (u32)(acc[i][j][r] + rqs[i][r] + cs);
+                            if (FULL || (cv && rbase + dr < B)) out[(u64)dr * tab_stride] = (float)dot;
+                        }
                     }
                 }
-            }
-        };
-        if (row0 + 64 <= B && t * 64 + 64 <= ncols) epilogue(std::true_type{});
-        else epilogue(std::false_type{});
-        if (!more) break;
-        store_tile(P ^ 1);
-        __syncthreads();
-        P ^= 1;
-        t += G;
+            };
+            if (row0 + 64 <= B && t * 64 + 64 <= ncols) epilogue(std::true_type{});
+            else epilogue(std::false_type{});
+            if (!more) break;
+            store_tile(P ^ 1);
+            __syncthreads();
+            P ^= 1;
+            t += 1;
+        }
     }
 }
 
@@ -986,24 +1003,23 @@
     return false;
 }
 template <int KC, bool Q2>
-static hipError_t launch_table_kc(dim3 grid, hipStream_t st, const uint8_t *qcodes, const u32 *qsums, u32 B, const uint8_t *tcodes, const u32 *tcsums,
-                                  u64 row_stride, u32 ncols, float *tab, u64 tab_stride) {
+static hipError_t launch_table_kc(u32 wgs, hipStream_t st, const uint8_t *qcodes, const u32 *qsums, u32 B, const uint8_t *tcodes, const u32 *tcsums,
+                                  u64 row_stride, u32 ncols, float *tab, u64 tab_stride, u32 *queue, u32 stripe) {
     const size_t lds = (size_t)2 * 64 * (KC * 64 + 16);
     hipError_t e = hipFuncSetAttribute((const void *)level_table_areg<KC, Q2>, hipFuncAttributeMaxDynamicSharedMemorySize, (int)lds);
     if (e != hipSuccess) return e;
-    hipLaunchKernelGGL((level_table_areg<KC, Q2>), grid, dim3(256), lds, st, qcodes, qsums, B, tcodes, tcsums, row_stride, ncols, tab, tab_stride);
+    hipLaunchKernelGGL((level_table_areg<KC, Q2>), dim3(wgs), dim3(256), lds, st, qcodes, qsums, B, tcodes, tcsums, row_stride, ncols, tab, tab_stride, queue, stripe);
     return hipGetLastError();
 }
 hipError_t launch_level_table_areg(int eng, u32 n_cus, hipStream_t st, const uint8_t *qcodes, const u32 *qsums, u32 B, const uint8_t *tcodes, const u32 *tcsums,
-                                   u64 row_stride, u32 ncols, float *tab, u64 tab_stride) {
-    const u32 n_tiles = (ncols + 63) / 64, row_groups = (B + 255) / 256;
-    const u32 G = std::max(1u, std::min(n_tiles, n_cus / std::max(1u, std::min(row_groups, n_cus))));
-    dim3 grid(G, row_groups);
+                                   u64 row_stride, u32 ncols, float *tab, u64 tab_stride, u32 *queue, u32 wgs, bool shared) {
+    const u32 stripe = table_gemm_stripe_tiles(B, ncols, n_cus, shared), n_items = table_gemm_items(B, ncols, n_cus, shared);
+    wgs = std::max(1u, std::min(n_items, wgs ? wgs : std::max(1u, n_cus)));
     const u32 kc = eng == ENG_Q2 ? (u32)(row_stride / 16) : (u32)(row_stride / 64);
-#define TAB_CASE(KC)                                                                                                                          \
-    case KC:                                                                                                                                  \
-        return eng == ENG_Q2 ? launch_table_kc<KC, true>(grid, st, qcodes, qsums, B, tcodes, tcsums, row_stride, ncols, tab, tab_stride)     \
-                             : launch_table_kc<KC, false>(grid, st, qcodes, qsums, B, tcodes, tcsums, row_stride, ncols, tab, tab_stride)
+#define TAB_CASE(KC)                                                                                                                                  \
+    case KC:                                                                                                                                          \
+        return eng == ENG_Q2 ? launch_table_kc<KC, true>(wgs, st, qcodes, qsums, B, tcodes, tcsums, row_stride, ncols, tab, tab_stride, queue, stripe) \
+                             : launch_table_kc<KC, false>(wgs, st, qcodes, qsums, B, tcodes, tcsums, row_stride, ncols, tab, tab_stride, queue, stripe)
     switch (kc) {
         TAB_CASE(2); TAB_CASE(4); TAB_CASE(6); TAB_CASE(8); TAB_CASE(12); TAB_CASE(16);
         default: return hipErrorInvalidValue;
diff --git a/cosdata_amd/csrc/kernels_walk.hip b/cosdata_amd/csrc/kernels_walk.hip
--- a/cosdata_amd/csrc/kernels_walk.hip
+++ b/cosdata_amd/csrc/kernels_walk.hip
@@ -15,7 +15,7 @@
 template <int ENG>
 __global__ __launch_bounds__(256) void quantize_rows_kernel(const float *__restrict__ x, u64 x_stride, u32 n, u32 dim, float lo,
                                                             float hi, uint8_t *__restrict__ codes, u64 row_stride,
-                                                            float *__restrict__ mags, float *__restrict__ raw_mags) {
+                                                            float *__restrict__ mags, float *__restrict__ raw_mags, u32 *__restrict__ code_sums) {
     const int lane = threadIdx.x & 63;
     const u32 row = blockIdx.x * (blockDim.x >> 6) + (threadIdx.x >> 6);
     if (row >= n) return;
@@ -26,7 +26,7 @@
     if (need_seq) rn = seq_norm_wave(xr, dim, lane);
     if (raw_mags && lane == 0) raw_mags[row] = rn;
     if constexpr (ENG == ENG_U8) {
-        u32 ss = 0;
+        u32 ss = 0, sum = 0;
         for (u32 i = lane; i < (u32)row_stride; i += 64) {
             uint8_t q = 0;
             if (i < dim) {
@@ -36,10 +36,16 @@
             }
             cr[i] = q;
             ss += (u32)q * (u32)q;
+            sum += (u32)q;
         }
 #pragma unroll
         for (int m = 32; m > 0; m >>= 1) ss += (u32)__shfl_xor((int)ss, m, 64);
         if (lane == 0) mags[row] = sqrtf((float)ss);
+        if (code_sums) {
+#pragma unroll
+            for (int m = 32; m > 0; m >>= 1) sum += (u32)__shfl_xor((int)sum, m, 64);
+            if (lane == 0) code_sums[row] = sum;
+        }
     } else if constexpr (ENG == ENG_Q2) {
         const u32 nch = (u32)(row_stride / 16);
         for (u32 c = 0; c < nch; c++) {
@@ -454,16 +460,16 @@
 namespace cosdev {
 
 hipError_t launch_quantize_rows(int eng, const float *x, u64 x_stride, u32 n, u32 dim, float lo, float hi, uint8_t *codes,
-                                u64 row_stride, float *mags, float *raw_mags, hipStream_t st) {
+                                u64 row_stride, float *mags, float *raw_mags, hipStream_t st, u32 *code_sums) {
     if (n == 0) return hipSuccess;
     dim3 block(256), grid((n + 3) / 4);
     switch (eng) {
-    case ENG_U8: hipLaunchKernelGGL(quantize_rows_kernel<ENG_U8>, grid, block, 0, st, x, x_stride, n, dim, lo, hi, codes, row_stride, mags, raw_mags); break;
-    case ENG_Q2: hipLaunchKernelGGL(quantize_rows_kernel<ENG_Q2>, grid, block, 0, st, x, x_stride, n, dim, lo, hi, codes, row_stride, mags, raw_mags); break;
-    case ENG_F32: hipLaunchKernelGGL(quantize_rows_kernel<ENG_F32>, grid, block, 0, st, x, x_stride, n, dim, lo, hi, codes, row_stride, mags, raw_mags); break;
-    case ENG_F16: hipLaunchKernelGGL(quantize_rows_kernel<ENG_F16>, grid, block, 0, st, x, x_stride, n, dim, lo, hi, codes, row_stride, mags, raw_mags); break;
-    case ENG_Q1: hipLaunchKernelGGL(quantize_rows_kernel<ENG_Q1>, grid, block, 0, st, x, x_stride, n, dim, lo, hi, codes, row_stride, mags, raw_mags); break;
-    case ENG_Q3: hipLaunchKernelGGL(quantize_rows_kernel<ENG_Q3>, grid, block, 0, st, x, x_stride, n, dim, lo, hi, codes, row_stride, mags, raw_mags); break;
+    case ENG_U8: hipLaunchKernelGGL(quantize_rows_kernel<ENG_U8>, grid, block, 0, st, x, x_stride, n, dim, lo, hi, codes, row_stride, mags, raw_mags, code_sums); break;
+    case ENG_Q2: hipLaunchKernelGGL(quantize_rows_kernel<ENG_Q2>, grid, block, 0, st, x, x_stride, n, dim, lo, hi, codes, row_stride, mags, raw_mags, code_sums); break;
+    case ENG_F32: hipLaunchKernelGGL(quantize_rows_kernel<ENG_F32>, grid, block, 0, st, x, x_stride, n, dim, lo, hi, codes, row_stride, mags, raw_mags, code_sums); break;
+    case ENG_F16: hipLaunchKernelGGL(quantize_rows_kernel<ENG_F16>, grid, block, 0, st, x, x_stride, n, dim, lo, hi, codes, row_stride, mags, raw_mags, code_sums); break;
+    case ENG_Q1: hipLaunchKernelGGL(quantize_rows_kernel<ENG_Q1>, grid, block, 0, st, x, x_stride, n, dim, lo, hi, codes, row_stride, mags, raw_mags, code_sums); break;
+    case ENG_Q3: hipLaunchKernelGGL(quantize_rows_kernel<ENG_Q3>, grid, block, 0, st, x, x_stride, n, dim, lo, hi, codes, row_stride, mags, raw_mags, code_sums); break;
     default: return hipErrorInvalidValue;
     }
     return hipGetLastError();
diff --git a/cosdata_amd/csrc/tuning.h b/cosdata_amd/csrc/tuning.h
--- a/cosdata_amd/csrc/tuning.h
+++ b/cosdata_amd/csrc/tuning.h
@@ -38,6 +38,7 @@
     TUNE_WALK_R2,
     TUNE_FINALIZE_WIDE_MAX_B,
     TUNE_FLAT_FP4_W8,
+    TUNE_WALK_TABLE_EARLY_WGS,
     TUNE_COUNT
 };
 
diff --git a/cosdata_amd/csrc/tuning.hip b/cosdata_amd/csrc/tuning.hip
--- a/cosdata_amd/csrc/tuning.hip
+++ b/cosdata_amd/csrc/tuning.hip
@@ -15,6 +15,7 @@
     "bm25_blocks", "sparse_layout", "walk_pb", "walk_pb_upper", "walk_lat", "walk_lat4", "walk_small_table_tk", "walk_lat_warm",
     "walk_lat_la", "walk_lat4_e", "finalize_fast", "shardset_force_rccl", "build_profile",
     "walk_merge_min", "walk_adj_mag", "walk_table_rule_c", "walk_table_after_sort", "walk_upper_lds_pad", "walk_r2", "finalize_wide_max_b", "flat_fp4_w8",
+    "walk_table_early_wgs",
 };
 std::atomic<long long> g_values[TUNE_COUNT];
 std::once_flag g_once;
diff --git a/cosdata_amd/csrc/walk_plan.h b/cosdata_amd/csrc/walk_plan.h
--- a/cosdata_amd/csrc/walk_plan.h
+++ b/cosdata_amd/csrc/walk_plan.h
@@ -33,6 +33,9 @@
     long long table_after_sort;
     bool table_supported;
     bool adj_mag_valid;
+    uint32_t table_early_wgs;
+    bool table_queue;
+    uint32_t n_cus;
 };
 
 struct WalkHave {
@@ -47,6 +50,7 @@
     bool ordered;
     bool use_table;
     bool table_waits_for_sort;
+    uint32_t table_early_wgs;
     uint32_t use_adj_mag;
     bool refill_adj_mag;
     bool chained;
@@ -54,6 +58,20 @@
     bool prepare_order, prepare_table;
     uint32_t table_level_min, table_cols, cut_after_level;
 };
+
+inline uint32_t table_gemm_stripe_tiles(uint32_t B, uint32_t cols, uint32_t n_cus, bool shared) {
+    const uint32_t n_tiles = (cols + 63u) / 64u, row_groups = (B + 255u) / 256u, cus = n_cus ? n_cus : 256u;
+    if (!shared) {
+        const uint32_t groups = std::max(1u, cus / std::max(1u, std::min(row_groups, cus)));
+        return std::max(1u, (n_tiles + groups - 1u) / groups);
+    }
+    const uint64_t units = (uint64_t)n_tiles * row_groups;
+    return (uint32_t)std::min<uint64_t>(64u, std::max<uint64_t>(2u, units / (24ull * cus)));
+}
+inline uint32_t table_gemm_items(uint32_t B, uint32_t cols, uint32_t n_cus, bool shared) {
+    const uint32_t n_tiles = (cols + 63u) / 64u, st = table_gemm_stripe_tiles(B, cols, n_cus, shared);
+    return (uint32_t)std::min<uint64_t>(0xFFFFFFFFull, (uint64_t)((n_tiles + st - 1u) / st) * ((B + 255u) / 256u));
+}
 
 inline bool walk_rows_over_64_slots(const WalkPlanIn &in) {
     for (uint32_t l = 0; l <= in.num_layers; l++)
@@ -107,6 +125,8 @@
         p.table_level_min = have->table_level_min;
         p.table_cols = have->table_cols;
         p.table_waits_for_sort = p.chained && (in.table_after_sort == 2 || (in.table_after_sort == 1 && (uint64_t)have->table_cols * in.B >= (1ull << 30)));
+        if (p.table_waits_for_sort && in.table_queue)
+            p.table_early_wgs = std::min(in.table_early_wgs, table_gemm_items(in.B, have->table_cols, in.n_cus, true));
     }
     if (have && p.ordered) p.cut_after_level = have->order_level0;
     if (in.adj_mag_valid && in.adj_mag_mode != 0)
diff --git a/include/cosdata_hip.h b/include/cosdata_hip.h
--- a/include/cosdata_hip.h
+++ b/include/cosdata_hip.h
@@ -135,7 +135,7 @@
     uint32_t table_level_min;
     uint32_t table_cols;
     uint32_t cut_after_level;
-    uint32_t reserved;
+    uint32_t table_early_wgs;
     float table_ms;
     float upper_ms, sort_ms, lower_ms;
     double table_int8_ops;
```

Measured after the change: 1.046 million (median of 6 runs). +2.5%, better.
